# zju3dv/Diffuman4D

Measured on NVIDIA H100. Metric: unet_window_denoise_steps_per_sec, higher is better.
Workload: dtype bf16

## Files before the change

diffuman4d_b200/_lib.py:

```python
from __future__ import annotations

import ctypes as C
import os

_HERE = os.path.dirname(os.path.abspath(__file__))
LIB_PATH = os.path.join(_HERE, "libd4d.so")

EXPORTS = [
    "d4d_last_error", "d4d_version", "d4d_create", "d4d_destroy", "d4d_load_weight", "d4d_finalize_weights",
    "d4d_num_weights", "d4d_weight_key", "d4d_unet_forward", "d4d_profile_forward", "d4d_workspace_bytes", "d4d_forward_launches",
    "d4d_denoise_window", "d4d_denoise_window_dpm", "d4d_assemble_input", "d4d_cfg_ddim_step", "d4d_cfg_dpm_step",
    "d4d_op_gemm", "d4d_op_gemm_kv_scatter", "d4d_op_conv3x3",
    "d4d_op_attention", "d4d_op_groupnorm", "d4d_op_conv3x3_groupnorm", "d4d_op_conv_resample", "d4d_op_layernorm", "d4d_op_pose_conv0", "d4d_op_pose_conv", "d4d_debug_tap", "d4d_exchange_alloc",
    "d4d_exchange_open", "d4d_unet_forward_sharded", "d4d_denoise_window_sharded", "d4d_denoise_window_dpm_sharded",
    "d4d_window_exchange", "d4d_op_window_scatter", "d4d_denoise_window_unipc", "d4d_cfg_unipc_step",
]


class D4DConfig(C.Structure):
    _fields_ = [
        ("in_channels", C.c_int32), ("out_channels", C.c_int32), ("block_out_channels", C.c_int32 * 4),
        ("layers_per_block", C.c_int32), ("num_heads", C.c_int32 * 4), ("has_attn2", C.c_int32 * 4),
        ("use_linear_projection", C.c_int32), ("norm_num_groups", C.c_int32), ("norm_eps", C.c_float),
        ("flip_sin_to_cos", C.c_int32), ("freq_shift", C.c_float), ("num_3d_attn_blocks", C.c_int32),
        ("enable_tem_embeds", C.c_int32), ("enable_pose_encoder", C.c_int32), ("center_input_sample", C.c_int32),
    ]


class D4DSched(C.Structure):
    _fields_ = [
        ("timesteps_table", C.c_void_p), ("alphas_cumprod", C.c_void_p), ("n_steps", C.c_int32),
        ("num_train_timesteps", C.c_int32), ("final_alpha_cumprod", C.c_float), ("prediction_type", C.c_int32),
        ("clip_sample", C.c_int32), ("clip_sample_range", C.c_float), ("emulate_bf16", C.c_int32),
    ]


class D4DDpmSched(C.Structure):
    _fields_ = [
        ("timesteps_table", C.c_void_p), ("coefs", C.c_void_p), ("n_steps", C.c_int32), ("prediction_type", C.c_int32),
        ("solver_order", C.c_int32), ("final_first_order", C.c_int32), ("emulate_bf16", C.c_int32),
    ]


class D4DUniPCSched(C.Structure):
    _fields_ = [
        ("timesteps_table", C.c_void_p), ("coefs", C.c_void_p), ("n_steps", C.c_int32), ("prediction_type", C.c_int32),
        ("solver_order", C.c_int32), ("emulate_bf16", C.c_int32),
    ]


class D4DError(RuntimeError):
    pass


_lib = None


def lib() -> C.CDLL:
    global _lib
    if _lib is None:
        _lib = _load(LIB_PATH)
    return _lib


def _load(path: str) -> C.CDLL:
    if not os.path.exists(path):
        raise ImportError(
            f"{path} not found: the CUDA extension is the product and there is no CPU fallback. "
            "Build it with `python -m diffuman4d_b200.build`.")
    l = C.CDLL(path)
    vp, i32, i64p, f32, f32p = C.c_void_p, C.c_int, C.POINTER(C.c_int64), C.c_float, C.c_void_p
    l.d4d_last_error.restype = C.c_char_p
    l.d4d_last_error.argtypes = []
    l.d4d_version.restype = C.c_int
    l.d4d_create.argtypes = [C.POINTER(D4DConfig), i32, C.POINTER(vp)]
    l.d4d_destroy.argtypes = [vp]
    l.d4d_destroy.restype = None
    l.d4d_load_weight.argtypes = [vp, C.c_char_p, vp, i64p, i32, i32]
    l.d4d_finalize_weights.argtypes = [vp]
    l.d4d_num_weights.argtypes = [vp]
    l.d4d_weight_key.argtypes = [vp, i32]
    l.d4d_weight_key.restype = C.c_char_p
    l.d4d_unet_forward.argtypes = [vp, vp, vp, vp, C.POINTER(C.c_int32), i32, i32, i32, i32, i32, vp, vp]
    l.d4d_profile_forward.argtypes = [vp, vp, vp, vp, C.POINTER(C.c_int32), i32, i32, i32, i32, i32, vp, vp,
                                      C.POINTER(C.c_float), C.POINTER(C.c_int32), C.POINTER(C.c_double)]
    l.d4d_workspace_bytes.argtypes = [vp, i32, i32, i32, i32, i32, C.POINTER(C.c_size_t)]
    l.d4d_forward_launches.argtypes = [vp, i32, i32, i32, i32, i32, C.POINTER(C.c_int)]
    l.d4d_denoise_window.argtypes = [vp, vp, vp, vp, vp, vp, vp, C.POINTER(D4DSched), f32, i32, i32, i32, i32, i32, vp]
    l.d4d_denoise_window_dpm.argtypes = [vp, vp, vp, vp, vp, vp, vp, C.POINTER(D4DDpmSched), f32, i32, i32, i32, i32, i32,
                                         vp, vp, vp]
    l.d4d_denoise_window_unipc.argtypes = [vp, vp, vp, vp, vp, vp, vp, C.POINTER(D4DUniPCSched), f32, i32, i32, i32, i32,
                                           i32, vp, vp, vp, vp, vp]
    l.d4d_assemble_input.argtypes = [vp, vp, vp, vp, vp, vp, vp, i32, i32, i32, i32, i32, vp, vp, vp]
    l.d4d_cfg_ddim_step.argtypes = [vp, vp, vp, vp, vp, C.POINTER(D4DSched), f32, i32, i32, i32, i32, vp, vp]
    l.d4d_cfg_dpm_step.argtypes = [vp, vp, vp, vp, vp, vp, vp, vp, C.POINTER(D4DDpmSched), f32, i32, i32, i32, i32, vp, vp]
    l.d4d_cfg_unipc_step.argtypes = [vp, vp, vp, vp, vp, vp, vp, vp, vp, vp, C.POINTER(D4DUniPCSched), f32, i32, i32, i32,
                                     i32, vp, vp]
    l.d4d_op_gemm.argtypes = [vp, i32, i32, vp, i32, i32, vp, i32, i32, f32p, vp, i32, i32, vp, i32, vp, i32, i32,
                              i32, f32, i32, vp, i32, vp]
    l.d4d_op_gemm_kv_scatter.argtypes = [vp, i32, i32, vp, i32, i32, vp, i32, i32, i32, C.c_int64, C.c_int64, C.c_int64,
                                         i32, vp, i32, vp]
    l.d4d_op_conv3x3.argtypes = [vp, i32, i32, i32, i32, vp, i32, f32p, vp, i32, vp, i32, vp, i32, vp, vp]
    l.d4d_op_attention.argtypes = [vp, vp, vp, i32, vp, i32, i32, i32, i32, i32, f32, i32, i32, vp]
    l.d4d_op_groupnorm.argtypes = [vp, i32, vp, i32, i32, i32, i32, f32, f32p, f32p, i32, vp, vp, vp]
    l.d4d_op_conv3x3_groupnorm.argtypes = [vp, i32, i32, i32, i32, vp, i32, f32p, vp, i32, f32, f32p, f32p, i32, vp, vp, vp,
                                           vp]
    l.d4d_op_conv_resample.argtypes = [vp, i32, i32, i32, i32, vp, i32, f32p, i32, i32, i32, vp, vp, vp]
    l.d4d_op_layernorm.argtypes = [vp, i32, i32, f32, f32p, f32p, vp, vp]
    l.d4d_op_pose_conv0.argtypes = [vp, i32, i32, i32, vp, f32p, vp, vp]
    l.d4d_op_pose_conv.argtypes = [vp, i32, i32, i32, i32, vp, f32p, i32, i32, i32, vp, vp]
    l.d4d_debug_tap.argtypes = [vp, vp, vp, vp, C.POINTER(C.c_int32), i32, i32, i32, i32, i32, i32, vp, C.c_char_p,
                                C.POINTER(C.c_int32), vp]
    l.d4d_exchange_alloc.argtypes = [vp, C.c_size_t, vp]
    l.d4d_exchange_open.argtypes = [vp, i32, i32, vp]
    l.d4d_unet_forward_sharded.argtypes = [vp, vp, vp, vp, C.POINTER(C.c_int32), i32, i32, i32, i32, i32, i32, vp, vp]
    l.d4d_denoise_window_sharded.argtypes = [vp, vp, vp, vp, vp, vp, vp, C.POINTER(D4DSched), f32, i32, i32, i32, i32,
                                             i32, i32, vp]
    l.d4d_denoise_window_dpm_sharded.argtypes = [vp, vp, vp, vp, vp, vp, vp, C.POINTER(D4DDpmSched), f32, i32, i32, i32,
                                                 i32, i32, i32, vp, vp, vp]
    l.d4d_window_exchange.argtypes = [vp, vp, vp, vp, vp, i32, i32, i32, i32, vp, vp, vp, vp, vp]
    l.d4d_op_window_scatter.argtypes = [vp, vp, vp, vp, i32, i32, i32, i32, i32, i32, vp, C.c_size_t, vp]
    for name in EXPORTS:
        fn = getattr(l, name)
        if fn.restype is C.c_int or name.startswith("d4d_op_") or name in (
                "d4d_create", "d4d_load_weight", "d4d_finalize_weights", "d4d_unet_forward", "d4d_denoise_window",
                "d4d_denoise_window_dpm", "d4d_exchange_alloc", "d4d_exchange_open", "d4d_unet_forward_sharded",
                "d4d_denoise_window_sharded", "d4d_denoise_window_dpm_sharded", "d4d_window_exchange", "d4d_debug_tap",
                "d4d_denoise_window_unipc"):
            fn.restype = C.c_int
    return l


def check(rc: int, what: str = ""):
    if rc == 0:
        return
    msg = lib().d4d_last_error().decode("utf-8", "replace")
    if rc == 1:
        raise ValueError(f"{what}: {msg}" if what else msg)
    raise D4DError(f"{what}: {msg} (status {rc})" if what else f"{msg} (status {rc})")
```

diffuman4d_b200/csrc/d4d_api.cu:

```cuda
#include <new>
#include <stdexcept>

#include "unet.h"

namespace d4d {
static thread_local std::string g_last_error;
void set_error(const std::string& msg) { g_last_error = msg; }
int nhwc_to_nchw_run(const bf16* x, int ld, int n, int C, int hw, bf16* out, cudaStream_t stream);
}

struct d4d_handle {
  d4d::Model* model;
};

using d4d::bf16;

#define D4D_API_BEGIN try {
#define D4D_API_END                                        \
  }                                                        \
  catch (const std::bad_alloc&) {                          \
    d4d::set_error("out of host memory");                  \
    return 2;                                              \
  }                                                        \
  catch (const std::exception& e) {                        \
    d4d::set_error(std::string("internal error: ") + e.what()); \
    return 2;                                              \
  }

namespace {
struct DeviceGuard {
  int prev = -1;
  bool ok = true;
  explicit DeviceGuard(int dev) {
    if (cudaGetDevice(&prev) != cudaSuccess) { ok = false; prev = -1; }
    if (ok && prev != dev && cudaSetDevice(dev) != cudaSuccess) ok = false;
  }
  ~DeviceGuard() {
    if (prev >= 0) cudaSetDevice(prev);
  }
};

int unet_forward(d4d_handle* h, const void* sample, const int64_t* timestep, const void* skeletons,
                 const int32_t* domain_ids, int n_domains, int B, int F, int F_total, int height, int width, void* out,
                 void* stream) {
  D4D_API_BEGIN
  D4D_REQUIRE(h != nullptr, "null handle");
  DeviceGuard g(h->model->device());
  return h->model->forward(static_cast<const bf16*>(sample), reinterpret_cast<const long long*>(timestep),
                           static_cast<const bf16*>(skeletons), domain_ids, n_domains, B, F, height, width,
                           static_cast<bf16*>(out), static_cast<cudaStream_t>(stream), F_total);
  D4D_API_END
}

int denoise_window(d4d_handle* h, void* latents, const void* pixel_latents, const void* plucker, const void* skeletons,
                   const void* cond_mask, int64_t* timestep_indices, const d4d::WindowStep& step, float guidance_scale,
                   int domain, int F, int F_total, int height, int width, int num_steps, void* stream) {
  D4D_API_BEGIN
  D4D_REQUIRE(h != nullptr && (step.ddim != nullptr || step.dpm != nullptr || step.unipc != nullptr), "null argument");
  DeviceGuard g(h->model->device());
  return h->model->denoise_window(static_cast<bf16*>(latents), static_cast<const bf16*>(pixel_latents),
                                  static_cast<const bf16*>(plucker), static_cast<const bf16*>(skeletons),
                                  static_cast<const bf16*>(cond_mask), reinterpret_cast<long long*>(timestep_indices),
                                  step, guidance_scale, domain, F, height, width, num_steps,
                                  static_cast<cudaStream_t>(stream), F_total);
  D4D_API_END
}

d4d::WindowStep ddim_step(const d4d_sched* sched) {
  d4d::WindowStep s;
  s.ddim = sched;
  return s;
}

d4d::WindowStep dpm_step(const d4d_dpm_sched* sched, void* x0_prev, int32_t* lower_order_nums) {
  d4d::WindowStep s;
  s.dpm = sched; s.x0_prev = static_cast<bf16*>(x0_prev); s.lower_order_nums = lower_order_nums;
  return s;
}
}

extern "C" {

const char* d4d_last_error(void) { return d4d::g_last_error.c_str(); }
int d4d_version(void) { return 107; }

int d4d_create(const d4d_config* cfg, int device, d4d_handle** out) {
  D4D_API_BEGIN
  D4D_REQUIRE(cfg != nullptr && out != nullptr, "null argument");
  *out = nullptr;
  D4D_REQUIRE(cfg->layers_per_block >= 1 && cfg->layers_per_block <= 4, "layers_per_block");
  D4D_REQUIRE(cfg->out_channels >= 1 && cfg->out_channels <= 16, "out_channels must be in [1,16]");
  D4D_REQUIRE(cfg->in_channels >= 1 && cfg->in_channels <= 16, "in_channels must be in [1,16]");
  D4D_REQUIRE(cfg->norm_num_groups >= 1 && cfg->norm_num_groups <= 64, "norm_num_groups");
  for (int i = 0; i < 4; ++i) {
    const int c = cfg->block_out_channels[i], hds = cfg->num_heads[i];
    D4D_REQUIRE(c > 0 && c % 64 == 0, "block_out_channels must be positive multiples of 64");
    D4D_REQUIRE(c % cfg->norm_num_groups == 0, "channels must be divisible by norm_num_groups");
    D4D_REQUIRE(hds > 0 && c % hds == 0, "channels must be divisible by the number of heads");
    D4D_REQUIRE(c / hds <= 192 && (c / hds) % 8 == 0, "head_dim must be a multiple of 8 and <= 192");
  }
  int ndev = 0;
  D4D_CUDA_OK(cudaGetDeviceCount(&ndev));
  D4D_REQUIRE(device >= 0 && device < ndev, "device index out of range");
  cudaDeviceProp prop;
  D4D_CUDA_OK(cudaGetDeviceProperties(&prop, device));
  if (prop.major != 9 || prop.minor != 0) {
    d4d::set_error("libd4d requires an sm_90a (Hopper H100) device; found compute capability " +
                   std::to_string(prop.major) + "." + std::to_string(prop.minor));
    return 2;
  }
  d4d_handle* h = new d4d_handle();
  h->model = new d4d::Model(*cfg, device);
  *out = h;
  return 0;
  D4D_API_END
}

void d4d_destroy(d4d_handle* h) {
  if (!h) return;
  try {
    delete h->model;
  } catch (...) {
  }
  delete h;
}

int d4d_load_weight(d4d_handle* h, const char* key, const void* data, const int64_t* shape, int ndim, int dtype) {
  D4D_API_BEGIN
  D4D_REQUIRE(h != nullptr, "null handle");
  return h->model->load_weight(key, data, shape, ndim, dtype);
  D4D_API_END
}

int d4d_finalize_weights(d4d_handle* h) {
  D4D_API_BEGIN
  D4D_REQUIRE(h != nullptr, "null handle");
  DeviceGuard g(h->model->device());
  return h->model->finalize();
  D4D_API_END
}

int d4d_num_weights(d4d_handle* h) { return h ? static_cast<int>(h->model->keys().size()) : 0; }
const char* d4d_weight_key(d4d_handle* h, int i) {
  if (!h || i < 0 || i >= static_cast<int>(h->model->keys().size())) return nullptr;
  return h->model->keys()[i].c_str();
}

int d4d_unet_forward(d4d_handle* h, const void* sample, const int64_t* timestep, const void* skeletons,
                     const int32_t* domain_ids, int n_domains, int B, int F, int height, int width, void* out,
                     void* stream) {
  return unet_forward(h, sample, timestep, skeletons, domain_ids, n_domains, B, F, 0, height, width, out, stream);
}

int d4d_profile_forward(d4d_handle* h, const void* sample, const int64_t* timestep, const void* skeletons,
                        const int32_t* domain_ids, int n_domains, int B, int F, int height, int width, void* out,
                        void* stream, float* ms_by_kind, int32_t* launches_by_kind, double* flops_by_kind) {
  D4D_API_BEGIN
  D4D_REQUIRE(h != nullptr, "null handle");
  DeviceGuard g(h->model->device());
  return h->model->profile(static_cast<const bf16*>(sample), reinterpret_cast<const long long*>(timestep),
                           static_cast<const bf16*>(skeletons), domain_ids, n_domains, B, F, height, width,
                           static_cast<bf16*>(out), static_cast<cudaStream_t>(stream), ms_by_kind, launches_by_kind,
                           flops_by_kind);
  D4D_API_END
}

int d4d_workspace_bytes(d4d_handle* h, int n_domains, int B, int F, int height, int width, size_t* bytes) {
  D4D_API_BEGIN
  D4D_REQUIRE(h != nullptr && bytes != nullptr, "null argument");
  d4d::Plan* p = h->model->find_plan(n_domains, B, F, height, width);
  *bytes = p ? p->arena_bytes : 0;
  return 0;
  D4D_API_END
}

int d4d_forward_launches(d4d_handle* h, int n_domains, int B, int F, int height, int width, int* launches) {
  D4D_API_BEGIN
  D4D_REQUIRE(h != nullptr && launches != nullptr, "null argument");
  d4d::Plan* p = h->model->find_plan(n_domains, B, F, height, width);
  *launches = p ? p->launches : 0;
  return 0;
  D4D_API_END
}

int d4d_denoise_window(d4d_handle* h, void* latents, const void* pixel_latents, const void* plucker,
                       const void* skeletons, const void* cond_mask, int64_t* timestep_indices, const d4d_sched* sched,
                       float guidance_scale, int domain, int F, int height, int width, int num_steps, void* stream) {
  return denoise_window(h, latents, pixel_latents, plucker, skeletons, cond_mask, timestep_indices, ddim_step(sched),
                        guidance_scale, domain, F, 0, height, width, num_steps, stream);
}

int d4d_denoise_window_dpm(d4d_handle* h, void* latents, const void* pixel_latents, const void* plucker,
                           const void* skeletons, const void* cond_mask, int64_t* timestep_indices,
                           const d4d_dpm_sched* sched, float guidance_scale, int domain, int F, int height, int width,
                           int num_steps, void* x0_prev, int32_t* lower_order_nums, void* stream) {
  return denoise_window(h, latents, pixel_latents, plucker, skeletons, cond_mask, timestep_indices,
                        dpm_step(sched, x0_prev, lower_order_nums), guidance_scale, domain, F, 0, height, width, num_steps,
                        stream);
}

int d4d_denoise_window_unipc(d4d_handle* h, void* latents, const void* pixel_latents, const void* plucker,
                             const void* skeletons, const void* cond_mask, int64_t* timestep_indices,
                             const d4d_unipc_sched* sched, float guidance_scale, int domain, int F, int height, int width,
                             int num_steps, void* x0_prev, void* x0_prev2, void* last_sample, int32_t* lower_order_nums,
                             void* stream) {
  d4d::WindowStep s;
  s.unipc = sched; s.x0_prev = static_cast<bf16*>(x0_prev); s.x0_prev2 = static_cast<bf16*>(x0_prev2);
  s.last_sample = static_cast<bf16*>(last_sample); s.lower_order_nums = lower_order_nums;
  return denoise_window(h, latents, pixel_latents, plucker, skeletons, cond_mask, timestep_indices, s, guidance_scale,
                        domain, F, 0, height, width, num_steps, stream);
}

int d4d_assemble_input(void* latents, const void* pixel_latents, const void* plucker, const void* skel_latents,
                       const void* cond_mask, const int64_t* timestep_indices, const int64_t* timesteps_table,
                       int n_steps, int F, int height, int width, int cfg, void* sample_out, int64_t* timestep_out,
                       void* stream) {
  D4D_API_BEGIN
  D4D_REQUIRE(latents && pixel_latents && plucker && cond_mask && timestep_indices && timesteps_table && sample_out &&
                  timestep_out, "null argument");
  d4d::AssembleArgs a;
  a.latents = static_cast<bf16*>(latents);
  a.pixel = static_cast<const bf16*>(pixel_latents);
  a.plucker = static_cast<const bf16*>(plucker);
  a.skel_latents = static_cast<const bf16*>(skel_latents);
  a.mask = static_cast<const bf16*>(cond_mask);
  a.timestep_indices = reinterpret_cast<const long long*>(timestep_indices);
  a.timesteps_table = reinterpret_cast<const long long*>(timesteps_table);
  a.n_steps = n_steps; a.F = F; a.h = height; a.w = width; a.cfg = cfg;
  a.sample = static_cast<bf16*>(sample_out);
  a.timestep_out = reinterpret_cast<long long*>(timestep_out);
  return d4d::assemble_input_run(a, static_cast<cudaStream_t>(stream));
  D4D_API_END
}

int d4d_cfg_ddim_step(const void* noise, const void* latents, const void* cond_mask, const int64_t* timestep_indices,
                      int64_t* timestep_indices_out, const d4d_sched* sched, float guidance_scale, int cfg, int F,
                      int height, int width, void* latents_out, void* stream) {
  D4D_API_BEGIN
  D4D_REQUIRE(noise && latents && cond_mask && timestep_indices && timestep_indices_out && sched && latents_out,
              "null argument");
  D4D_REQUIRE(timestep_indices != timestep_indices_out, "timestep_indices_out must not alias timestep_indices");
  d4d::DdimArgs d;
  const int hw = height * width;
  d.noise = static_cast<const bf16*>(noise); d.latents = static_cast<const bf16*>(latents);
  d.mask = static_cast<const bf16*>(cond_mask);
  d.timestep_indices = reinterpret_cast<const long long*>(timestep_indices);
  d.timesteps_table = reinterpret_cast<const long long*>(sched->timesteps_table);
  d.alphas_cumprod = sched->alphas_cumprod;
  d.n_steps = sched->n_steps; d.T = sched->num_train_timesteps; d.final_alpha_cumprod = sched->final_alpha_cumprod;
  d.F = F; d.chw = 4 * hw; d.hw = hw; d.cfg = cfg; d.guidance = guidance_scale;
  d.prediction_type = sched->prediction_type; d.clip_sample = sched->clip_sample; d.clip_range = sched->clip_sample_range;
  d.emulate_bf16 = sched->emulate_bf16; d.out = static_cast<bf16*>(latents_out);
  return d4d::cfg_ddim_step_run(d, reinterpret_cast<long long*>(timestep_indices_out), static_cast<cudaStream_t>(stream));
  D4D_API_END
}

int d4d_cfg_dpm_step(const void* noise, const void* latents, const void* cond_mask, const int64_t* timestep_indices,
                     int64_t* timestep_indices_out, void* x0_prev, const int32_t* lower_order_nums,
                     int32_t* lower_order_nums_out, const d4d_dpm_sched* sched, float guidance_scale, int cfg, int F,
                     int height, int width, void* latents_out, void* stream) {
  D4D_API_BEGIN
  D4D_REQUIRE(noise && latents && cond_mask && timestep_indices && timestep_indices_out && x0_prev && lower_order_nums &&
                  lower_order_nums_out && sched && sched->timesteps_table && sched->coefs && latents_out,
              "null argument");
  d4d::DpmArgs d;
  const int hw = height * width;
  d.noise = static_cast<const bf16*>(noise); d.latents = static_cast<const bf16*>(latents);
  d.mask = static_cast<const bf16*>(cond_mask);
  d.timestep_indices = reinterpret_cast<const long long*>(timestep_indices);
  d.coefs = sched->coefs; d.n_steps = sched->n_steps;
  d.F = F; d.chw = 4 * hw; d.hw = hw; d.cfg = cfg; d.guidance = guidance_scale;
  d.prediction_type = sched->prediction_type; d.solver_order = sched->solver_order;
  d.final_first_order = sched->final_first_order; d.emulate_bf16 = sched->emulate_bf16;
  d.x0_prev = static_cast<bf16*>(x0_prev); d.lower_order_nums = lower_order_nums;
  d.lower_order_nums_out = lower_order_nums_out; d.out = static_cast<bf16*>(latents_out);
  return d4d::cfg_dpm_step_run(d, reinterpret_cast<long long*>(timestep_indices_out), static_cast<cudaStream_t>(stream));
  D4D_API_END
}

int d4d_cfg_unipc_step(const void* noise, const void* latents, const void* cond_mask, const int64_t* timestep_indices,
                       int64_t* timestep_indices_out, void* x0_prev, void* x0_prev2, void* last_sample,
                       const int32_t* lower_order_nums, int32_t* lower_order_nums_out, const d4d_unipc_sched* sched,
                       float guidance_scale, int cfg, int F, int height, int width, void* latents_out, void* stream) {
  D4D_API_BEGIN
  D4D_REQUIRE(noise && latents && cond_mask && timestep_indices && timestep_indices_out && x0_prev && last_sample &&
                  lower_order_nums && lower_order_nums_out && sched && sched->timesteps_table && sched->coefs && latents_out,
              "null argument");
  d4d::UniPCArgs d;
  const int hw = height * width;
  d.noise = static_cast<const bf16*>(noise); d.latents = static_cast<const bf16*>(latents);
  d.mask = static_cast<const bf16*>(cond_mask);
  d.timestep_indices = reinterpret_cast<const long long*>(timestep_indices);
  d.coefs = sched->coefs; d.n_steps = sched->n_steps;
  d.F = F; d.chw = 4 * hw; d.hw = hw; d.cfg = cfg; d.guidance = guidance_scale;
  d.prediction_type = sched->prediction_type; d.solver_order = sched->solver_order; d.emulate_bf16 = sched->emulate_bf16;
  d.x0_prev = static_cast<bf16*>(x0_prev); d.x0_prev2 = static_cast<bf16*>(x0_prev2);
  d.last_sample = static_cast<bf16*>(last_sample); d.lower_order_nums = lower_order_nums;
  d.lower_order_nums_out = lower_order_nums_out; d.out = static_cast<bf16*>(latents_out);
  return d4d::cfg_unipc_step_run(d, reinterpret_cast<long long*>(timestep_indices_out), static_cast<cudaStream_t>(stream));
  D4D_API_END
}

int d4d_op_gemm(const void* A, int lda, int K1, const void* A2, int lda2, int K2, const void* W, int M, int N,
                const float* bias, const void* rowvec, int ld_rowvec, int rows_per_image, const void* residual,
                int ld_res, void* out, int ldo, int geglu, int act, float out_scale, int block_n, int64_t* stats,
                int stats_rows, void* stream) {
  D4D_API_BEGIN
  d4d::GemmDesc d;
  d.A = static_cast<const bf16*>(A); d.lda = lda; d.K1 = K1;
  d.A2 = static_cast<const bf16*>(A2); d.lda2 = lda2; d.K2 = K2;
  d.Wt = static_cast<const bf16*>(W); d.M = M; d.N = N; d.bias = bias;
  d.rowvec = static_cast<const bf16*>(rowvec); d.ld_rowvec = ld_rowvec; d.rows_per_image = rows_per_image;
  d.residual = static_cast<const bf16*>(residual); d.ld_res = ld_res;
  d.out = static_cast<bf16*>(out); d.ldo = ldo; d.geglu = geglu; d.act = act; d.out_scale = out_scale; d.block_n = block_n;
  d.stats = reinterpret_cast<long long*>(stats); d.stats_rows = stats_rows;
  D4D_REQUIRE(M > 0, "empty GEMM");
  d4d::GemmLaunch L;
  if (int rc = d4d::gemm_prepare(d, &L)) return rc;
  return d4d::gemm_run(L, static_cast<cudaStream_t>(stream));
  D4D_API_END
}

int d4d_op_gemm_kv_scatter(const void* A, int lda, int K, const void* W, int M, int N, void* out, int ldo, int kv_col0,
                           int kv_ld, int64_t rows_local, int64_t rows_global, int64_t row_offset, int world,
                           void* const* kv_dst, int block_n, void* stream) {
  D4D_API_BEGIN
  D4D_REQUIRE(M > 0, "empty GEMM");
  D4D_REQUIRE(world >= 1 && world <= 8, "K/V scatter: world must be in [1, 8]");
  D4D_REQUIRE(kv_dst != nullptr, "K/V scatter: null destination buffer");
  d4d::GemmDesc d;
  d.A = static_cast<const bf16*>(A); d.lda = lda; d.K1 = K; d.Wt = static_cast<const bf16*>(W); d.M = M; d.N = N;
  d.out = static_cast<bf16*>(out); d.ldo = ldo; d.block_n = block_n;
  d.kv_world = world; d.kv_col0 = kv_col0; d.kv_ld = kv_ld;
  d.kv_rows_local = rows_local; d.kv_rows_global = rows_global; d.kv_row_offset = row_offset;
  for (int r = 0; r < world; ++r) d.kv_dst[r] = static_cast<bf16*>(kv_dst[r]);
  d4d::GemmLaunch L;
  if (int rc = d4d::gemm_prepare(d, &L)) return rc;
  return d4d::gemm_run(L, static_cast<cudaStream_t>(stream));
  D4D_API_END
}

int d4d_op_conv3x3(const void* x_nhwc, int n_img, int H, int W, int Cin, const void* Wt, int Cout, const float* bias,
                   const void* rowvec, int ld_rowvec, const void* residual, int act, void* out, int block_n,
                   int64_t* stats, void* stream) {
  D4D_API_BEGIN
  D4D_REQUIRE(n_img > 0 && H > 0 && W > 0, "empty conv");
  d4d::GemmDesc d;
  d.conv = 1; d.A = static_cast<const bf16*>(x_nhwc); d.n_img = n_img; d.H = H; d.W = W; d.Cin = Cin;
  d.Wt = static_cast<const bf16*>(Wt); d.N = Cout; d.bias = bias;
  d.rowvec = static_cast<const bf16*>(rowvec); d.ld_rowvec = ld_rowvec;
  d.residual = static_cast<const bf16*>(residual); d.ld_res = Cout;
  d.out = static_cast<bf16*>(out); d.ldo = Cout; d.act = act; d.block_n = block_n;
  d.stats = reinterpret_cast<long long*>(stats);
  d4d::GemmLaunch L;
  if (int rc = d4d::gemm_prepare(d, &L)) return rc;
  return d4d::gemm_run(L, static_cast<cudaStream_t>(stream));
  D4D_API_END
}

int d4d_op_attention(const void* q, const void* k, const void* v, int ld_qkv, void* out, int ld_out, int batch, int seq,
                     int heads, int head_dim, float scale, int seq_kv, int ld_kv, void* stream) {
  D4D_API_BEGIN
  d4d::AttnDesc d;
  d.q = static_cast<const bf16*>(q); d.k = static_cast<const bf16*>(k); d.v = static_cast<const bf16*>(v);
  d.ld_qkv = ld_qkv; d.out = static_cast<bf16*>(out); d.ld_out = ld_out;
  d.batch = batch; d.seq = seq; d.heads = heads; d.head_dim = head_dim; d.scale = scale;
  d.seq_kv = seq_kv; d.ld_kv = ld_kv;
  d4d::AttnLaunch L;
  if (int rc = d4d::attn_prepare(d, &L)) return rc;
  return d4d::attn_run(L, static_cast<cudaStream_t>(stream));
  D4D_API_END
}

int d4d_op_groupnorm(const void* x1, int C1, const void* x2, int C2, int n_img, int hw, int groups, float eps,
                     const float* gamma, const float* beta, int silu, void* out, int64_t* stats, void* stream) {
  D4D_API_BEGIN
  D4D_REQUIRE(n_img > 0 && hw > 0 && groups > 0, "empty GroupNorm");
  cudaStream_t st = static_cast<cudaStream_t>(stream);
  if (x2 == nullptr) C2 = 0;
  long long* s1 = reinterpret_cast<long long*>(stats);
  long long* s2 = C2 > 0 ? s1 + static_cast<size_t>(n_img) * C1 * 2 : nullptr;
  if (int rc = d4d::groupnorm_stats_run(static_cast<const bf16*>(x1), C1, n_img, hw, s1, st)) return rc;
  if (C2 > 0) {
    if (int rc = d4d::groupnorm_stats_run(static_cast<const bf16*>(x2), C2, n_img, hw, s2, st)) return rc;
  }
  return d4d::groupnorm_apply_run(static_cast<const bf16*>(x1), C1, s1, static_cast<const bf16*>(x2), C2, s2, n_img, hw, groups,
                                  eps, gamma, beta, silu, static_cast<bf16*>(out), st);
  D4D_API_END
}

int d4d_op_conv_resample(const void* x_nhwc, int n_img, int H, int W, int Cin, const void* Wt, int Cout, const float* bias,
                         int kind, int up_a, int up_b, void* out, int64_t* stats, void* stream) {
  D4D_API_BEGIN
  D4D_REQUIRE(n_img > 0 && H > 0 && W > 0 && kind >= 1 && kind <= 3, "conv_resample arguments");
  d4d::GemmDesc d;
  d.conv = 1; d.conv_kind = kind; d.up_a = up_a; d.up_b = up_b;
  d.A = static_cast<const bf16*>(x_nhwc); d.n_img = n_img; d.H = H; d.W = W; d.Cin = Cin;
  d.Wt = static_cast<const bf16*>(Wt); d.N = Cout; d.bias = bias;
  d.out = static_cast<bf16*>(out); d.ldo = Cout;
  d.stats = reinterpret_cast<long long*>(stats);
  d4d::GemmLaunch L;
  if (int rc = d4d::gemm_prepare(d, &L)) return rc;
  return d4d::gemm_run(L, static_cast<cudaStream_t>(stream));
  D4D_API_END
}

int d4d_op_conv3x3_groupnorm(const void* x_nhwc, int n_img, int H, int W, int Cin, const void* Wt, int Cout, const float* bias,
                             const void* residual, int groups, float eps, const float* gamma, const float* beta, int silu,
                             void* conv_out, void* gn_out, int64_t* stats, void* stream) {
  D4D_API_BEGIN
  D4D_REQUIRE(n_img > 0 && H > 0 && W > 0 && groups > 0, "empty conv");
  D4D_REQUIRE(stats != nullptr, "null statistics workspace");
  cudaStream_t st = static_cast<cudaStream_t>(stream);
  d4d::GemmDesc d;
  d.conv = 1; d.A = static_cast<const bf16*>(x_nhwc); d.n_img = n_img; d.H = H; d.W = W; d.Cin = Cin;
  d.Wt = static_cast<const bf16*>(Wt); d.N = Cout; d.bias = bias;
  d.residual = static_cast<const bf16*>(residual); d.ld_res = Cout;
  d.out = static_cast<bf16*>(conv_out); d.ldo = Cout;
  d.stats = reinterpret_cast<long long*>(stats);
  d4d::GemmLaunch L;
  if (int rc = d4d::gemm_prepare(d, &L)) return rc;
  if (int rc = d4d::gemm_run(L, st)) return rc;
  return d4d::groupnorm_apply_run(static_cast<const bf16*>(conv_out), Cout, d.stats, nullptr, 0, nullptr, n_img, H * W, groups, eps,
                                  gamma, beta, silu, static_cast<bf16*>(gn_out), st);
  D4D_API_END
}

int d4d_op_layernorm(const void* x, int rows, int C, float eps, const float* gamma, const float* beta, void* out,
                     void* stream) {
  D4D_API_BEGIN
  return d4d::layernorm_run(static_cast<const bf16*>(x), rows, C, eps, gamma, beta, static_cast<bf16*>(out),
                            static_cast<cudaStream_t>(stream));
  D4D_API_END
}

int d4d_op_pose_conv0(const void* x_nchw, int n, int H, int W, const void* Wt, const float* bias, void* out_nhwc4,
                      void* stream) {
  D4D_API_BEGIN
  D4D_REQUIRE(n > 0 && H > 0 && W > 0, "empty pose conv");
  return d4d::pose_conv0_run(static_cast<const bf16*>(x_nchw), n, H, W, static_cast<const bf16*>(Wt), bias,
                             static_cast<bf16*>(out_nhwc4), static_cast<cudaStream_t>(stream));
  D4D_API_END
}

int d4d_op_pose_conv(const void* x_nhwc, int n, int Cin, int H, int W, const void* Wt, const float* bias, int Cout,
                     int ksize, int stride, void* out, void* stream) {
  D4D_API_BEGIN
  D4D_REQUIRE(n > 0 && H > 0 && W > 0, "empty pose conv");
  return d4d::pose_conv_run(static_cast<const bf16*>(x_nhwc), n, Cin, H, W, static_cast<const bf16*>(Wt), bias, Cout,
                            ksize, stride, static_cast<bf16*>(out), static_cast<cudaStream_t>(stream));
  D4D_API_END
}

int d4d_debug_tap(d4d_handle* h, const void* sample, const int64_t* timestep, const void* skeletons,
                  const int32_t* domain_ids, int n_domains, int B, int F, int height, int width, int tap, void* out,
                  char* name64, int32_t* dims3, void* stream) {
  D4D_API_BEGIN
  D4D_REQUIRE(h != nullptr, "null handle");
  DeviceGuard g(h->model->device());
  return h->model->debug_tap(static_cast<const bf16*>(sample), reinterpret_cast<const long long*>(timestep),
                             static_cast<const bf16*>(skeletons), domain_ids, n_domains, B, F, height, width, tap,
                             static_cast<bf16*>(out), name64, dims3, static_cast<cudaStream_t>(stream));
  D4D_API_END
}

int d4d_unet_forward_sharded(d4d_handle* h, const void* sample, const int64_t* timestep, const void* skeletons,
                             const int32_t* domain_ids, int n_domains, int B_local, int F_local, int F_total, int height,
                             int width, void* out, void* stream) {
  return unet_forward(h, sample, timestep, skeletons, domain_ids, n_domains, B_local, F_local, F_total, height, width,
                      out, stream);
}

int d4d_denoise_window_sharded(d4d_handle* h, void* latents, const void* pixel_latents, const void* plucker,
                               const void* skeletons, const void* cond_mask, int64_t* timestep_indices,
                               const d4d_sched* sched, float guidance_scale, int domain, int F_local, int F_total,
                               int height, int width, int num_steps, void* stream) {
  return denoise_window(h, latents, pixel_latents, plucker, skeletons, cond_mask, timestep_indices, ddim_step(sched),
                        guidance_scale, domain, F_local, F_total, height, width, num_steps, stream);
}

int d4d_denoise_window_dpm_sharded(d4d_handle* h, void* latents, const void* pixel_latents, const void* plucker,
                                   const void* skeletons, const void* cond_mask, int64_t* timestep_indices,
                                   const d4d_dpm_sched* sched, float guidance_scale, int domain, int F_local, int F_total,
                                   int height, int width, int num_steps, void* x0_prev, int32_t* lower_order_nums,
                                   void* stream) {
  return denoise_window(h, latents, pixel_latents, plucker, skeletons, cond_mask, timestep_indices,
                        dpm_step(sched, x0_prev, lower_order_nums), guidance_scale, domain, F_local, F_total, height,
                        width, num_steps, stream);
}

int d4d_window_exchange(d4d_handle* h, const void* latents_local, const int64_t* timestep_indices_local,
                        const void* x0_prev_local, const int32_t* lower_order_nums_local, int F_local, int F_total,
                        int height, int width, void* latents_out, int64_t* timestep_indices_out, void* x0_prev_out,
                        int32_t* lower_order_nums_out, void* stream) {
  D4D_API_BEGIN
  D4D_REQUIRE(h != nullptr, "null handle");
  DeviceGuard g(h->model->device());
  return h->model->window_exchange(static_cast<const bf16*>(latents_local),
                                   reinterpret_cast<const long long*>(timestep_indices_local),
                                   static_cast<const bf16*>(x0_prev_local), lower_order_nums_local, F_local, F_total, height,
                                   width, static_cast<bf16*>(latents_out), reinterpret_cast<long long*>(timestep_indices_out),
                                   static_cast<bf16*>(x0_prev_out), lower_order_nums_out, static_cast<cudaStream_t>(stream));
  D4D_API_END
}

int d4d_op_window_scatter(const void* latents, const int64_t* timestep_indices, const void* x0_prev,
                          const int32_t* lower_order_nums, int F_local, int F_total, int height, int width, int world,
                          int rank, void* const* dst, size_t dst_bytes, void* stream) {
  D4D_API_BEGIN
  D4D_REQUIRE(world >= 1 && world <= 8, "window scatter: world must be in [1, 8]");
  D4D_REQUIRE(dst != nullptr, "window scatter: null destination buffer");
  D4D_REQUIRE(height > 0 && width > 0, "window scatter: latent height/width");
  d4d::WindowScatterArgs a;
  for (int r = 0; r < 8; ++r) a.dst[r] = r < world ? dst[r] : nullptr;
  a.world = world; a.rank = rank; a.F_local = F_local; a.F_total = F_total;
  a.chw = 4ll * height * width;
  a.latents = static_cast<const bf16*>(latents); a.ts = reinterpret_cast<const long long*>(timestep_indices);
  a.x0_prev = static_cast<const bf16*>(x0_prev); a.lower_order_nums = lower_order_nums;
  return d4d::window_scatter_run(a, dst_bytes, static_cast<cudaStream_t>(stream));
  D4D_API_END
}

int d4d_exchange_alloc(d4d_handle* h, size_t kv_bytes, unsigned char* handles_out) {
  D4D_API_BEGIN
  D4D_REQUIRE(h != nullptr, "null handle");
  DeviceGuard g(h->model->device());
  return h->model->exchange_alloc(kv_bytes, handles_out);
  D4D_API_END
}

int d4d_exchange_open(d4d_handle* h, int rank, int world, const unsigned char* all_handles) {
  D4D_API_BEGIN
  D4D_REQUIRE(h != nullptr, "null handle");
  DeviceGuard g(h->model->device());
  return h->model->exchange_open(rank, world, all_handles);
  D4D_API_END
}

}
```

diffuman4d_b200/csrc/gemm_wgmma.cu:

```cuda
#include "kernels.h"
#include "wgmma.cuh"

namespace d4d {

namespace {

constexpr int BLOCK_M = 128;
constexpr int BLOCK_K = 64;
constexpr int A_BYTES = BLOCK_M * BLOCK_K * 2;
constexpr int BAR_BYTES = 1024;
constexpr int NUM_THREADS = 384;
constexpr int MAX_SMEM = 227 * 1024;

constexpr int SLAB_COLS = 32;
constexpr int SLAB_BYTES = 64 * SLAB_COLS * 2;

template <int BN, bool kStaged>
struct GemmCfg {
  static constexpr int STAGE_BYTES = A_BYTES + BN * BLOCK_K * 2;
  static constexpr int STAGING_BYTES = kStaged ? 2 * 64 * BN * 2 : 0;
  static constexpr int STAGES_FIT = (MAX_SMEM - 1024 - BAR_BYTES - STAGING_BYTES) / STAGE_BYTES;
  static constexpr int STAGES = STAGES_FIT > 8 ? 8 : STAGES_FIT;
  static constexpr int SMEM = 1024 + BAR_BYTES + STAGES * STAGE_BYTES + STAGING_BYTES;
};

struct TileCoord {
  int m0;
  int n_img0, y0, x0;
  int pa, pb;
};

template <bool kConv>
__device__ __forceinline__ void tile_coords(const GemmKernelArgs& a, int m_tile, TileCoord& t) {
  if (!kConv) {
    t.m0 = m_tile * BLOCK_M;
    t.n_img0 = t.y0 = t.x0 = 0;
    t.pa = t.pb = 0;
  } else {
    const int ph = a.n_phases > 1 ? m_tile / a.tiles_per_phase : 0;
    m_tile -= ph * a.tiles_per_phase;
    t.pa = ph >> 1;
    t.pb = ph & 1;
    int tx = m_tile % a.tiles_x;
    int r = m_tile / a.tiles_x;
    int ty = r % a.tiles_y;
    int tn = r / a.tiles_y;
    t.m0 = 0;
    t.x0 = tx * a.BW;
    t.y0 = ty * a.BH;
    t.n_img0 = tn * a.BN;
  }
}

template <bool kConv>
__device__ __forceinline__ void row_of(const GemmKernelArgs& a, const TileCoord& tc, int rr, long long& row, int& img,
                                       bool& valid) {
  if (!kConv) {
    row = static_cast<long long>(tc.m0) + rr;
    valid = row < a.M;
    img = a.rows_per_image > 0 ? static_cast<int>(row / a.rows_per_image) : 0;
  } else {
    const int bx = rr % a.BW;
    const int r2 = rr / a.BW;
    const int by = r2 % a.BH;
    const int bn = r2 / a.BH;
    const int x = tc.x0 + bx, y = tc.y0 + by, n = tc.n_img0 + bn;
    valid = (x < a.W) && (y < a.H) && (n < a.n_img);
    row = (static_cast<long long>(n) * a.out_H + (y * a.out_sy + a.out_oy + tc.pa)) * a.out_W + (x * a.out_sx + a.out_ox + tc.pb);
    img = n;
  }
}

enum : int { E_BIAS = 1, E_ROWVEC = 2, E_ACT = 4, E_RES = 8, E_STATS = 16, E_KV = 32, E_ALL = 63 };
__host__ __device__ constexpr bool gemm_staged(bool conv, int epi) { return !conv && !(epi & E_KV); }

template <int BN, bool kGeglu, bool kConv, int kEpi>
__global__ void __launch_bounds__(NUM_THREADS, 1)
gemm_wgmma_kernel(const __grid_constant__ CUtensorMap tmap_a, const __grid_constant__ CUtensorMap tmap_a2,
                  const __grid_constant__ CUtensorMap tmap_b, const __grid_constant__ CUtensorMap tmap_c,
                  const __grid_constant__ CUtensorMap tmap_r, const GemmKernelArgs a) {
  constexpr bool kStaged = gemm_staged(kConv, kEpi);
  using Cfg = GemmCfg<BN, kStaged>;
  constexpr int STAGES = Cfg::STAGES;
  extern __shared__ uint8_t smem_raw[];
  uint8_t* smem = reinterpret_cast<uint8_t*>((reinterpret_cast<uintptr_t>(smem_raw) + 1023) & ~uintptr_t(1023));
  uint64_t* full = reinterpret_cast<uint64_t*>(smem);
  uint64_t* empty = full + STAGES;
  uint64_t* res_full = empty + STAGES;
  uint8_t* ring = smem + BAR_BYTES;

  const int warp = __shfl_sync(0xffffffffu, threadIdx.x >> 5, 0);
  const int lane = threadIdx.x & 31;
  const int total_tiles = a.m_tiles * a.n_tiles;

  if (threadIdx.x == 0) {
    tma_prefetch_desc(&tmap_a);
    tma_prefetch_desc(&tmap_b);
    if (a.kb_split < a.k_blocks) tma_prefetch_desc(&tmap_a2);
    for (int i = 0; i < STAGES; ++i) {
      mbar_init(&full[i], 1);
      mbar_init(&empty[i], 2);
    }
    mbar_init(&res_full[0], 1);
    mbar_init(&res_full[1], 1);
    fence_mbar_init();
  }
  __syncthreads();
  pdl_wait();
  pdl_launch_dependents();

  if (warp < 4) {
    setmaxnreg_dec<40>();
    if (threadIdx.x == 0) {
      const uint32_t tx_bytes = A_BYTES + static_cast<uint32_t>(a.block_n) * BLOCK_K * 2;
      int stage = 0;
      uint32_t phase = 0;
      for (int tile = blockIdx.x; tile < total_tiles; tile += gridDim.x) {
        const int m_tile = tile / a.n_tiles;
        const int n_tile = tile % a.n_tiles;
        TileCoord tc;
        tile_coords<kConv>(a, m_tile, tc);
        const int n0 = n_tile * a.block_n;
        for (int kb = 0; kb < a.k_blocks; ++kb) {
          mbar_wait(&empty[stage], phase ^ 1);
          uint8_t* sa = ring + stage * Cfg::STAGE_BYTES;
          uint8_t* sb = sa + A_BYTES;
          mbar_expect_tx(&full[stage], tx_bytes);
          if (!kConv) {
            if (kb < a.kb_split) tma_load_2d(sa, &tmap_a, &full[stage], kb * BLOCK_K, tc.m0);
            else tma_load_2d(sa, &tmap_a2, &full[stage], (kb - a.kb_split) * BLOCK_K, tc.m0);
            tma_load_2d(sb, &tmap_b, &full[stage], kb * BLOCK_K, n0);
          } else {
            const int tap = kb / a.cin_blocks;
            const int cb = kb - tap * a.cin_blocks;
            tma_load_4d(sa, &tmap_a, &full[stage], cb * BLOCK_K, tc.x0 * a.in_stride + a.tap_dx[tap] + tc.pb,
                        tc.y0 * a.in_stride + a.tap_dy[tap] + tc.pa, tc.n_img0);
            tma_load_2d(sb, &tmap_b, &full[stage], tap * a.Cin + cb * BLOCK_K, n0 + (tc.pa * 2 + tc.pb) * a.N);
          }
          if (++stage == STAGES) { stage = 0; phase ^= 1; }
        }
      }
    }
    return;
  }

  setmaxnreg_inc<232>();
  const int wg = (warp >> 2) - 1;
  const int wq = warp & 3;
  const bool wg_leader = (threadIdx.x & 127) == 0;
  const int r_base = wg * 64 + wq * 16 + (lane >> 2);
  const int c_base = 2 * (lane & 3);
  const uint32_t ring_u32 = smem_u32(ring);
  const bool staged = kStaged && a.staged;
  uint8_t* stg = ring + STAGES * Cfg::STAGE_BYTES + wg * 64 * BN * 2;
  const uint32_t stg_u32 = smem_u32(stg) + (r_base - wg * 64) * 64 + c_base * 2;
  const int stg_xor = (lane >> 3) & 3;
  const bool has_res = (kEpi & E_RES) && !kGeglu && a.residual != nullptr;
  const int out_cols = kGeglu ? a.N / 2 : a.N;
  uint32_t res_phase = 0;

  int stage = 0;
  uint32_t phase = 0;
  float acc[BN / 2];
  for (int tile = blockIdx.x; tile < total_tiles; tile += gridDim.x) {
    const int m_tile = tile / a.n_tiles;
    const int n_tile = tile % a.n_tiles;
    TileCoord tc;
    tile_coords<kConv>(a, m_tile, tc);
    const int n0 = n_tile * a.block_n;
    const int ocol0 = kGeglu ? n0 / 2 : n0;
    const int ocols = min(kGeglu ? a.block_n / 2 : a.block_n, out_cols - ocol0);
    const int n_slabs = (ocols + SLAB_COLS - 1) / SLAB_COLS;
    const int orow0 = tc.m0 + wg * 64;
    const bool stg_live = staged && orow0 < a.M;

    int prev_stage = -1;
    for (int kb = 0; kb < a.k_blocks; ++kb) {
      mbar_wait(&full[stage], phase);
      const uint32_t sa = ring_u32 + stage * Cfg::STAGE_BYTES + wg * 64 * 128;
      const uint32_t sb = ring_u32 + stage * Cfg::STAGE_BYTES + A_BYTES;
      const uint64_t adesc = make_wgmma_desc(sa, 16, 1024);
      const uint64_t bdesc = make_wgmma_desc(sb, 16, 1024);
      wgmma_fence();
#pragma unroll
      for (int k = 0; k < BLOCK_K / 16; ++k) {
        const int scale_d = (kb | k) != 0 ? 1 : 0;
        if constexpr (BN == 64) wgmma_ss_n64(acc, adesc + 2 * k, bdesc + 2 * k, scale_d);
        else if constexpr (BN == 128) wgmma_ss_n128(acc, adesc + 2 * k, bdesc + 2 * k, scale_d);
        else if constexpr (BN == 160) wgmma_ss_n160(acc, adesc + 2 * k, bdesc + 2 * k, scale_d);
        else if constexpr (BN == 192) wgmma_ss_n192(acc, adesc + 2 * k, bdesc + 2 * k, scale_d);
        else wgmma_ss_n256(acc, adesc + 2 * k, bdesc + 2 * k, scale_d);
      }
      wgmma_commit();
      if (kb == 0 && staged && wg_leader) {
        bulk_wait_group_read<0>();
        if (has_res && stg_live) {
          mbar_expect_tx(&res_full[wg], n_slabs * SLAB_BYTES);
          for (int s = 0; s < n_slabs; ++s)
            tma_load_2d(stg + s * SLAB_BYTES, &tmap_r, &res_full[wg], ocol0 + s * SLAB_COLS, orow0);
        }
      }
      wgmma_wait<1>();
      if (prev_stage >= 0 && wg_leader) mbar_arrive(&empty[prev_stage]);
      prev_stage = stage;
      if (++stage == STAGES) { stage = 0; phase ^= 1; }
    }
    wgmma_wait<0>();
    wgmma_fence_regs(acc);
    if (wg_leader) mbar_arrive(&empty[prev_stage]);

    long long rows[2];
    int imgs[2];
    bool valid[2];
    row_of<kConv>(a, tc, r_base, rows[0], imgs[0], valid[0]);
    row_of<kConv>(a, tc, r_base + 8, rows[1], imgs[1], valid[1]);
    if (staged) {
      named_barrier_sync(1 + wg, 128);
      if (has_res && stg_live) {
        mbar_wait(&res_full[wg], res_phase);
        res_phase ^= 1;
      }
    }
    auto stg_addr = [&](int j, int h) {
      return stg_u32 + h * 8 * 64 + (j >> 2) * SLAB_BYTES + (((j & 3) ^ stg_xor) << 4);
    };

    if constexpr (kGeglu) {
      const bool has_bias = (kEpi & E_BIAS) && a.bias != nullptr;
#pragma unroll
      for (int p = 0; p < BN / 16; ++p) {
        if (16 * p >= a.block_n || n0 + 16 * p >= a.N) break;
        float2 ba = make_float2(0.f, 0.f), bg = make_float2(0.f, 0.f);
        if (has_bias) {
          ba = __ldg(reinterpret_cast<const float2*>(a.bias + n0 + 16 * p + c_base));
          bg = __ldg(reinterpret_cast<const float2*>(a.bias + n0 + 16 * p + 8 + c_base));
        }
        const int ocol = n0 / 2 + 8 * p + c_base;
#pragma unroll
        for (int h = 0; h < 2; ++h) {
          if (!valid[h]) continue;
          const float a0 = acc[8 * p + 2 * h] + ba.x, a1 = acc[8 * p + 2 * h + 1] + ba.y;
          const float g0 = acc[8 * p + 4 + 2 * h] + bg.x, g1 = acc[8 * p + 4 + 2 * h + 1] + bg.y;
          const uint32_t o = pack_bf16x2(a0 * gelu_erf_f(g0), a1 * gelu_erf_f(g1));
          if (staged) st_shared_u32(stg_addr(p, h), o);
          else *reinterpret_cast<uint32_t*>(a.out + static_cast<size_t>(rows[h]) * a.ldo + ocol) = o;
        }
      }
    } else {
      const bool has_bias = (kEpi & E_BIAS) && a.bias != nullptr, has_rv = (kEpi & E_ROWVEC) && a.rowvec != nullptr;
      const bool has_stats = (kEpi & E_STATS) && a.stats != nullptr;
      const bool has_act = (kEpi & E_ACT) && a.act == 1, has_scale = (kEpi & E_ACT) && a.out_scale != 1.0f;
      const bool has_kv = (kEpi & E_KV) && a.kv_world > 0;
      const long long row0 = __shfl_sync(0xffffffffu, rows[0], 0);
      const bool stats_on = has_stats && __shfl_sync(0xffffffffu, valid[0] ? 1 : 0, 0);
      const int stats_img = !kConv ? static_cast<int>(row0 / a.stats_rows) : __shfl_sync(0xffffffffu, imgs[0], 0);
#pragma unroll
      for (int j = 0; j < BN / 8; ++j) {
        const int cl = 8 * j + c_base;
        const int col = n0 + cl;
        if (8 * j >= a.block_n || n0 + 8 * j >= a.N) break;
        float2 b2 = make_float2(0.f, 0.f);
        if (has_bias) b2 = __ldg(reinterpret_cast<const float2*>(a.bias + col));
        float sv[2][2];
#pragma unroll
        for (int h = 0; h < 2; ++h) {
          sv[h][0] = sv[h][1] = 0.f;
          if (!valid[h]) continue;
          float f0 = acc[4 * j + 2 * h] + b2.x, f1 = acc[4 * j + 2 * h + 1] + b2.y;
          if (has_rv) {
            const float2 v = unpack_bf16x2(*reinterpret_cast<const uint32_t*>(a.rowvec + static_cast<size_t>(imgs[h]) * a.ld_rowvec + col));
            f0 += v.x; f1 += v.y;
          }
          if (has_act) { f0 = silu_f(f0); f1 = silu_f(f1); }
          if (has_scale) { f0 *= a.out_scale; f1 *= a.out_scale; }
          if (has_res) {
            const float2 v = unpack_bf16x2(staged ? ld_shared_u32(stg_addr(j, h))
                                                  : *reinterpret_cast<const uint32_t*>(a.residual + static_cast<size_t>(rows[h]) * a.ld_res + col));
            f0 += v.x; f1 += v.y;
          }
          const uint32_t o = pack_bf16x2(f0, f1);
          if (has_stats) {
            const float2 rv = unpack_bf16x2(o);
            sv[h][0] = rv.x; sv[h][1] = rv.y;
          }
          if (has_kv && col >= a.kv_col0) {
            const long long half = rows[h] / a.kv_rows_local;
            const long long grow = half * a.kv_rows_global + a.kv_row_offset + (rows[h] - half * a.kv_rows_local);
            const size_t off = static_cast<size_t>(grow) * a.kv_ld + (col - a.kv_col0);
#pragma unroll 1
            for (int rk = 0; rk < a.kv_world; ++rk) *reinterpret_cast<uint32_t*>(a.kv_dst[rk] + off) = o;
          } else if (staged) {
            st_shared_u32(stg_addr(j, h), o);
          } else {
            *reinterpret_cast<uint32_t*>(a.out + static_cast<size_t>(rows[h]) * a.ldo + col) = o;
          }
        }
        if (has_stats) {
          float s0 = sv[0][0] + sv[1][0], s1 = sv[0][1] + sv[1][1];
          float q0 = sv[0][0] * sv[0][0] + sv[1][0] * sv[1][0], q1 = sv[0][1] * sv[0][1] + sv[1][1] * sv[1][1];
#pragma unroll
          for (int m = 4; m < 32; m <<= 1) {
            s0 += __shfl_xor_sync(0xffffffffu, s0, m);
            s1 += __shfl_xor_sync(0xffffffffu, s1, m);
            q0 += __shfl_xor_sync(0xffffffffu, q0, m);
            q1 += __shfl_xor_sync(0xffffffffu, q1, m);
          }
          if (stats_on && lane < 4) {
            unsigned long long* st = reinterpret_cast<unsigned long long*>(a.stats) + (static_cast<size_t>(stats_img) * a.N + col) * 2;
            atomicAdd(st + 0, static_cast<unsigned long long>(__float2ll_rn(s0 * kGnSumScale)));
            atomicAdd(st + 1, static_cast<unsigned long long>(__float2ll_rn(q0 * kGnSqScale)));
            atomicAdd(st + 2, static_cast<unsigned long long>(__float2ll_rn(s1 * kGnSumScale)));
            atomicAdd(st + 3, static_cast<unsigned long long>(__float2ll_rn(q1 * kGnSqScale)));
          }
        }
      }
    }
    if (staged) {
      fence_proxy_async_smem();
      named_barrier_sync(1 + wg, 128);
      if (wg_leader && stg_live) {
        for (int s = 0; s < n_slabs; ++s) tma_store_2d(&tmap_c, stg + s * SLAB_BYTES, ocol0 + s * SLAB_COLS, orow0);
        bulk_commit_group();
      }
    }
  }
  if (staged && wg_leader) bulk_wait_group<0>();
}

}

int gemm_prepare(const GemmDesc& d, GemmLaunch* L) {
  D4D_REQUIRE(d.N % 16 == 0, "GEMM N must be a multiple of 16");
  D4D_REQUIRE(d.out != nullptr && d.A != nullptr && d.Wt != nullptr, "null operand");
  D4D_REQUIRE(d.kv_world >= 0 && d.kv_world <= 8, "K/V scatter: world must be in [1, 8]");
  if (d.kv_world > 0) {
    D4D_REQUIRE(!d.conv && !d.geglu && d.kv_col0 >= 0 && d.kv_col0 < d.N && d.kv_col0 % 16 == 0 && d.kv_ld % 8 == 0 &&
                d.kv_ld >= d.N - d.kv_col0, "K/V scatter arguments");
    for (int r = 0; r < d.kv_world; ++r) D4D_REQUIRE(d.kv_dst[r] != nullptr, "K/V scatter: null destination buffer");
    D4D_REQUIRE(d.kv_rows_local > 0 && d.M % d.kv_rows_local == 0, "K/V scatter: M must be a multiple of rows_local");
    D4D_REQUIRE(d.kv_row_offset >= 0 && d.kv_row_offset + d.kv_rows_local <= d.kv_rows_global,
                "K/V scatter: row_offset + rows_local exceeds rows_global");
  }
  GemmKernelArgs& a = L->args;
  memset(&a, 0, sizeof(a));
  int dev = 0, sms = 0;
  D4D_CUDA_OK(cudaGetDevice(&dev));
  D4D_CUDA_OK(cudaDeviceGetAttribute(&sms, cudaDevAttrMultiProcessorCount, dev));
  int bn = d.block_n;
  if (bn <= 0) {
    const long long rows = d.conv ? static_cast<long long>(d.n_img) * d.H * d.W : d.M;
    const long long m_tiles_est = (rows + BLOCK_M - 1) / BLOCK_M;
    long long best_cost = -1;
    for (int c : {64, 128, 160, 192, 256}) {
      if (d.geglu && c % 64 != 0) continue;
      const long long tiles = m_tiles_est * ((d.N + c - 1) / c);
      const long long waves = (tiles + sms - 1) / sms;
      const long long cost = waves * (c + 64) + (static_cast<long long>((d.N + c - 1) / c) * c - d.N) / 4;
      if (best_cost < 0 || cost <= best_cost) { best_cost = cost; bn = c; }
    }
  }
  D4D_REQUIRE(bn >= 16 && bn <= 256 && bn % 16 == 0 && (d.block_n <= 0 || d.N % bn == 0), "no valid block_n");
  a.block_n = bn;
  a.n_tiles = (d.N + bn - 1) / bn;
  a.N = d.N;
  a.bias = d.bias;
  a.rowvec = d.rowvec;
  a.ld_rowvec = d.ld_rowvec;
  a.rows_per_image = d.rows_per_image;
  a.residual = d.residual;
  a.ld_res = d.ld_res;
  a.out = d.out;
  a.ldo = d.ldo;
  a.geglu = d.geglu;
  a.act = d.act;
  a.out_scale = d.out_scale;
  a.stats = d.stats;
  a.stats_rows = d.stats_rows > 0 ? d.stats_rows : 1;
  D4D_REQUIRE(d.stats == nullptr || (!d.geglu && d.kv_world == 0), "GroupNorm statistics: plain / conv epilogue only");
  D4D_REQUIRE(d.stats == nullptr || d.conv || (d.stats_rows > 0 && d.stats_rows % 32 == 0), "statistics need rows-per-image % 32 == 0");
  D4D_REQUIRE(d.stats == nullptr || d.conv || d.M % d.stats_rows == 0, "statistics need M % rows-per-image == 0");
  a.kv_world = d.kv_world;
  a.kv_col0 = d.kv_col0;
  a.kv_ld = d.kv_ld;
  a.kv_rows_local = d.kv_rows_local > 0 ? d.kv_rows_local : 1;
  a.kv_rows_global = d.kv_rows_global;
  a.kv_row_offset = d.kv_row_offset;
  for (int i = 0; i < 8; ++i) a.kv_dst[i] = d.kv_dst[i];
  D4D_REQUIRE(d.ldo % 8 == 0 && (d.residual == nullptr || d.ld_res % 8 == 0) &&
              (d.rowvec == nullptr || d.ld_rowvec % 8 == 0), "leading dimensions must be multiples of 8");

  if (!d.conv) {
    D4D_REQUIRE(d.K1 > 0 && d.K1 % 8 == 0 && d.K2 % 8 == 0, "K must be a multiple of 8");
    D4D_REQUIRE(d.A2 == nullptr || d.K1 % BLOCK_K == 0, "two-source GEMM needs K1 % 64 == 0");
    a.mode = 0;
    a.M = d.M;
    a.m_tiles = (d.M + BLOCK_M - 1) / BLOCK_M;
    a.kb_split = (d.K1 + BLOCK_K - 1) / BLOCK_K;
    const int kb2 = d.A2 ? (d.K2 + BLOCK_K - 1) / BLOCK_K : 0;
    a.k_blocks = a.kb_split + kb2;
    const int K = d.K1 + (d.A2 ? d.K2 : 0);
    if (int rc = make_tmap_2d(&L->tmap_a, d.A, d.M, d.K1, d.lda, BLOCK_K, BLOCK_M, 128)) return rc;
    if (d.A2) {
      if (int rc = make_tmap_2d(&L->tmap_a2, d.A2, d.M, d.K2, d.lda2, BLOCK_K, BLOCK_M, 128)) return rc;
    } else {
      L->tmap_a2 = L->tmap_a;
    }
    if (int rc = make_tmap_2d(&L->tmap_b, d.Wt, d.N, K, K, BLOCK_K, bn, 128)) return rc;
    const auto aligned16 = [](const void* p) { return (reinterpret_cast<uintptr_t>(p) & 15) == 0; };
    a.staged = d.kv_world == 0 && (d.geglu ? bn % (2 * SLAB_COLS) : bn % SLAB_COLS) == 0 && aligned16(d.out) &&
               (d.residual == nullptr || aligned16(d.residual));
    L->tmap_c = L->tmap_r = L->tmap_a;
    if (a.staged) {
      if (int rc = make_tmap_2d(&L->tmap_c, d.out, d.M, d.geglu ? d.N / 2 : d.N, d.ldo, SLAB_COLS, 64, 64)) return rc;
      if (d.residual && !d.geglu)
        if (int rc = make_tmap_2d(&L->tmap_r, d.residual, d.M, d.N, d.ld_res, SLAB_COLS, 64, 64)) return rc;
    }
  } else {
    D4D_REQUIRE(d.Cin % 8 == 0, "conv Cin must be a multiple of 8");
    D4D_REQUIRE(d.conv_kind >= 0 && d.conv_kind <= 3, "conv_kind");
    D4D_REQUIRE(d.conv_kind != 1 || (d.H % 2 == 0 && d.W % 2 == 0), "stride-2 conv needs even H, W");
    a.mode = 1;
    a.n_img = d.n_img; a.Cin = d.Cin;
    a.in_stride = 1; a.out_sy = a.out_sx = 1; a.out_oy = a.out_ox = 0;
    a.n_phases = 1;
    if (d.conv_kind >= 2) {
      const int pa = d.conv_kind == 3 ? 0 : d.up_a, pb = d.conv_kind == 3 ? 0 : d.up_b;
      a.n_taps = 4;
      for (int t = 0; t < 4; ++t) {
        a.tap_dy[t] = static_cast<signed char>((t >> 1) + pa - 1);
        a.tap_dx[t] = static_cast<signed char>((t & 1) + pb - 1);
      }
      a.H = d.H; a.W = d.W; a.out_H = 2 * d.H; a.out_W = 2 * d.W;
      a.out_sy = a.out_sx = 2; a.out_oy = pa; a.out_ox = pb;
      if (d.conv_kind == 3) a.n_phases = 4;
    } else {
      a.n_taps = 9;
      for (int t = 0; t < 9; ++t) {
        a.tap_dy[t] = static_cast<signed char>(t / 3 - 1);
        a.tap_dx[t] = static_cast<signed char>(t % 3 - 1);
      }
      if (d.conv_kind == 1) { a.in_stride = 2; a.H = d.H / 2; a.W = d.W / 2; }
      else { a.H = d.H; a.W = d.W; }
      a.out_H = a.H; a.out_W = a.W;
    }
    a.M = d.n_img * a.H * a.W;
    a.cin_blocks = (d.Cin + BLOCK_K - 1) / BLOCK_K;
    a.k_blocks = a.n_taps * a.cin_blocks;
    a.kb_split = a.k_blocks;
    int bw = 16; while (bw > a.W) bw >>= 1;
    int bh = 128 / bw; while (bh > a.H && bh > 1) bh >>= 1;
    int bnimg = 128 / (bw * bh);
    D4D_REQUIRE(bw * bh * bnimg == 128 && bnimg <= 256, "conv tile shape");
    D4D_REQUIRE(d.stats == nullptr || (bw * bh) % 32 == 0, "statistics need 32-row warps inside one image");
    a.BW = bw; a.BH = bh; a.BN = bnimg;
    a.tiles_x = (a.W + bw - 1) / bw;
    a.tiles_y = (a.H + bh - 1) / bh;
    const int tiles_n = (d.n_img + bnimg - 1) / bnimg;
    a.tiles_per_phase = a.tiles_x * a.tiles_y * tiles_n;
    a.m_tiles = a.tiles_per_phase * a.n_phases;
    a.M *= a.n_phases;
    if (int rc = make_tmap_nhwc(&L->tmap_a, d.A, d.n_img, d.H, d.W, d.Cin, BLOCK_K, bw, bh, bnimg, 128, a.in_stride)) return rc;
    L->tmap_a2 = L->tmap_c = L->tmap_r = L->tmap_a;
    const uint64_t kw = static_cast<uint64_t>(a.n_taps) * d.Cin;
    if (int rc = make_tmap_2d(&L->tmap_b, d.Wt, static_cast<uint64_t>(d.N) * a.n_phases, kw, kw, BLOCK_K, bn, 128)) return rc;
  }
  const int total = a.m_tiles * a.n_tiles;
  L->grid = total < sms ? total : sms;
  return 0;
}

namespace {

using GemmKernelFn = void (*)(const CUtensorMap, const CUtensorMap, const CUtensorMap, const CUtensorMap,
                              const CUtensorMap, const GemmKernelArgs);
struct GemmVariant {
  int bn;
  bool geglu, conv;
  int epi;
  GemmKernelFn fn;
  int smem;
};
#define D4D_GV(BN, G, C, E) {BN, G, C, E, gemm_wgmma_kernel<BN, G, C, E>, GemmCfg<BN, gemm_staged(C, E)>::SMEM}
#define D4D_GV_PLAIN(BN)                                                                                              \
                                         \
  D4D_GV(BN, false, false, 0), D4D_GV(BN, false, false, E_BIAS), D4D_GV(BN, false, false, E_BIAS | E_RES),           \
  D4D_GV(BN, false, false, E_BIAS | E_RES | E_STATS), D4D_GV(BN, false, false, E_ALL)
#define D4D_GV_CONV(BN)                                                                                               \
                                                            \
  D4D_GV(BN, false, true, E_BIAS | E_ROWVEC | E_STATS), D4D_GV(BN, false, true, E_BIAS | E_RES | E_STATS),           \
  D4D_GV(BN, false, true, E_BIAS | E_STATS), D4D_GV(BN, false, true, E_ALL)
const GemmVariant kGemmVariants[] = {
    D4D_GV_PLAIN(128), D4D_GV_CONV(128), D4D_GV(128, true, false, E_BIAS),
    D4D_GV_PLAIN(160), D4D_GV_CONV(160),
    D4D_GV_PLAIN(192),
    D4D_GV_PLAIN(256), D4D_GV_CONV(256), D4D_GV(256, true, false, E_BIAS),
    D4D_GV(64, false, false, E_ALL), D4D_GV(64, false, true, E_ALL), D4D_GV(64, true, false, E_BIAS),
};
#undef D4D_GV_CONV
#undef D4D_GV_PLAIN
#undef D4D_GV
constexpr int kNumGemmVariants = sizeof(kGemmVariants) / sizeof(kGemmVariants[0]);

int gemm_variant_at(const GemmKernelArgs& a, int bn) {
  const bool conv = a.mode != 0, geglu = a.geglu != 0;
  int need = 0;
  if (a.bias) need |= E_BIAS;
  if (!geglu) {
    if (a.rowvec) need |= E_ROWVEC;
    if (a.act == 1 || a.out_scale != 1.0f) need |= E_ACT;
    if (a.residual) need |= E_RES;
    if (a.stats) need |= E_STATS;
    if (a.kv_world > 0) need |= E_KV;
  }
  int generic = -1;
  for (int i = 0; i < kNumGemmVariants; ++i) {
    const GemmVariant& v = kGemmVariants[i];
    if (v.bn != bn || v.geglu != geglu || v.conv != conv) continue;
    if (v.epi == need) return i;
    if ((v.epi & need) == need && (generic < 0 || v.epi == E_ALL)) generic = i;
  }
  return generic;
}

int gemm_variant_of(const GemmKernelArgs& a) {
  for (int bn : {64, 128, 160, 192, 256}) {
    if (bn < a.block_n) continue;
    const int vi = gemm_variant_at(a, bn);
    if (vi >= 0) return vi;
  }
  return -1;
}

}

int gemm_run(const GemmLaunch& L, cudaStream_t stream) {
  static PerDeviceOnce attr_once[kNumGemmVariants];
  const int vi = gemm_variant_of(L.args);
  D4D_REQUIRE(vi >= 0, "no GEMM kernel instantiation covers this launch");
  const GemmVariant& v = kGemmVariants[vi];
  if (int rc = ensure_dyn_smem(v.fn, v.smem, attr_once[vi])) return rc;
  D4D_CUDA_OK(launch_pdl(v.fn, dim3(L.grid), dim3(NUM_THREADS), v.smem, stream, L.tmap_a, L.tmap_a2, L.tmap_b, L.tmap_c, L.tmap_r,
                         L.args));
  D4D_CUDA_OK(cudaGetLastError());
  return 0;
}

double gemm_flops(const GemmLaunch& L) {
  return 2.0 * static_cast<double>(L.args.M) * L.args.N * (static_cast<double>(L.args.k_blocks) * BLOCK_K);
}

}
```

diffuman4d_b200/csrc/kernels.h:

```cpp
#pragma once
#include <cstdlib>
#include <mutex>
#include <utility>
#include <string.h>

#include "common.cuh"

namespace d4d {

constexpr float kGnSumScale = 268435456.f;
constexpr float kGnSqScale = 16777216.f;

struct GemmKernelArgs {
  int M, N, k_blocks, block_n, n_tiles, m_tiles;
  int mode;
  int kb_split;
  int H, W, n_img, Cin, cin_blocks, BW, BH, BN, tiles_x, tiles_y;
  int n_taps, in_stride, out_sy, out_sx, out_oy, out_ox, out_H, out_W;
  int n_phases, tiles_per_phase;
  signed char tap_dy[9], tap_dx[9];
  const float* bias;
  const bf16* rowvec;
  int ld_rowvec, rows_per_image;
  const bf16* residual;
  int ld_res;
  bf16* out;
  int ldo;
  int staged;
  int geglu;
  int act;
  float out_scale;
  long long* stats;
  int stats_rows;
  int kv_world, kv_col0, kv_ld;
  long long kv_rows_local, kv_rows_global, kv_row_offset;
  bf16* kv_dst[8];
};

struct GemmDesc {
  const bf16* A = nullptr;
  int lda = 0, K1 = 0;
  const bf16* A2 = nullptr;
  int lda2 = 0, K2 = 0;
  const bf16* Wt = nullptr;
  int M = 0, N = 0;
  const float* bias = nullptr;
  const bf16* rowvec = nullptr;
  int ld_rowvec = 0, rows_per_image = 0;
  const bf16* residual = nullptr;
  int ld_res = 0;
  bf16* out = nullptr;
  int ldo = 0;
  int geglu = 0;
  int act = 0;
  float out_scale = 1.0f;
  int block_n = 0;
  long long* stats = nullptr;
  int stats_rows = 0;
  int kv_world = 0, kv_col0 = 0, kv_ld = 0;
  long long kv_rows_local = 0, kv_rows_global = 0, kv_row_offset = 0;
  bf16* kv_dst[8] = {nullptr, nullptr, nullptr, nullptr, nullptr, nullptr, nullptr, nullptr};
  int conv = 0, n_img = 0, H = 0, W = 0, Cin = 0;
  int conv_kind = 0, up_a = 0, up_b = 0;
};

struct GemmLaunch {
  CUtensorMap tmap_a, tmap_a2, tmap_b, tmap_c, tmap_r;
  GemmKernelArgs args;
  int grid;
};

int gemm_prepare(const GemmDesc& d, GemmLaunch* L);
int gemm_run(const GemmLaunch& L, cudaStream_t stream);
double gemm_flops(const GemmLaunch& L);

struct AttnDesc {
  const bf16* q = nullptr;
  const bf16* k = nullptr;
  const bf16* v = nullptr;
  int ld_qkv = 0;
  bf16* out = nullptr;
  int ld_out = 0;
  int batch = 0, seq = 0, heads = 0, head_dim = 0;
  int seq_kv = 0;
  int ld_kv = 0;
  float scale = 0.f;
};
struct AttnLaunch {
  CUtensorMap tmap_q, tmap_k, tmap_v;
  AttnDesc d;
  int grid_x, grid_y;
  int variant;
};
int attn_prepare(const AttnDesc& d, AttnLaunch* L);
int attn_run(const AttnLaunch& L, cudaStream_t stream);
double attn_flops(const AttnDesc& d);

int groupnorm_stats_run(const bf16* x, int C, int n_img, int hw, long long* stats, cudaStream_t stream);
int groupnorm_apply_run(const bf16* x1, int C1, const long long* stats1, const bf16* x2, int C2, const long long* stats2, int n_img,
                        int hw, int groups, float eps, const float* gamma, const float* beta, int silu, bf16* out,
                        cudaStream_t stream);
int layernorm_run(const bf16* x, int rows, int C, float eps, const float* gamma, const float* beta, bf16* out,
                  cudaStream_t stream);

int sinusoid_run(const float* pos, int n, int dim, int flip, float freq_shift, bf16* out, cudaStream_t stream);
int sinusoid_i64_run(const long long* pos, int n, int dim, int flip, float freq_shift, bf16* out, cudaStream_t stream);
int silu_run(const bf16* x, long long n, bf16* out, cudaStream_t stream);
int im2col_nchw_run(const bf16* x, int n, int Cin, int H, int W, int cin_pad, int KP, bf16* out, cudaStream_t stream);
int nhwc_to_nchw_run(const bf16* x, int ld, int n, int C, int hw, bf16* out, cudaStream_t stream);
int pose_conv0_run(const bf16* x_nchw, int n, int H, int W, const bf16* w, const float* bias, bf16* out_nhwc4,
                   cudaStream_t stream);
int pose_conv_run(const bf16* x, int n, int Cin, int H, int W, const bf16* w, const float* bias, int Cout, int ksize,
                  int stride, bf16* out_nhwc, cudaStream_t stream);
int im2col_nhwc_run(const bf16* x, int n, int H, int W, int C, int ksize, int stride, bf16* out, cudaStream_t stream);

struct AssembleArgs {
  bf16* latents;
  const bf16* pixel;
  const bf16* plucker;
  const bf16* skel_latents;
  const bf16* mask;
  const long long* timestep_indices;
  const long long* timesteps_table;
  int n_steps;
  int F, h, w, cfg;
  bf16* sample;
  long long* timestep_out;
};
int assemble_input_run(const AssembleArgs& a, cudaStream_t stream);

struct DdimArgs {
  const bf16* noise;
  const bf16* latents;
  const bf16* mask;
  const long long* timestep_indices;
  const long long* timesteps_table;
  const float* alphas_cumprod;
  int n_steps, T;
  float final_alpha_cumprod;
  int F, chw, hw, cfg;
  float guidance;
  int prediction_type;
  int clip_sample;
  float clip_range;
  int emulate_bf16;
  bf16* out;
};
int cfg_ddim_step_run(const DdimArgs& a, long long* ts_out, cudaStream_t stream);

constexpr int kDpmCoefs = 6;
struct DpmArgs {
  const bf16* noise;
  const bf16* latents;
  const bf16* mask;
  const long long* timestep_indices;
  const float* coefs;
  int n_steps;
  int F, chw, hw, cfg;
  float guidance;
  int prediction_type;
  int solver_order;
  int final_first_order;
  int emulate_bf16;
  bf16* x0_prev;
  const int* lower_order_nums;
  int* lower_order_nums_out;
  bf16* out;
};
int cfg_dpm_step_run(const DpmArgs& a, long long* ts_out, cudaStream_t stream);

constexpr int kUniPCCoefs = 14;
struct UniPCArgs {
  const bf16* noise;
  const bf16* latents;
  const bf16* mask;
  const long long* timestep_indices;
  const float* coefs;
  int n_steps;
  int F, chw, hw, cfg;
  float guidance;
  int prediction_type;
  int solver_order;
  int emulate_bf16;
  bf16* x0_prev;
  bf16* x0_prev2;
  bf16* last_sample;
  const int* lower_order_nums;
  int* lower_order_nums_out;
  bf16* out;
};
int cfg_unipc_step_run(const UniPCArgs& a, long long* ts_out, cudaStream_t stream);

struct KvFlagArgs {
  unsigned int* flags[8];
  int rank, world;
  unsigned int epoch;
  int slot;
};
int kv_signal_run(const KvFlagArgs& a, cudaStream_t stream);
int kv_wait_run(const KvFlagArgs& a, cudaStream_t stream);

struct WindowResultLayout {
  size_t x0, ts, lon, bytes;
};
inline WindowResultLayout window_result_layout(long long F_total, long long chw, bool dpm) {
  WindowResultLayout L;
  const size_t rows = static_cast<size_t>(F_total) * static_cast<size_t>(chw) * 2;
  L.x0 = rows;
  L.ts = dpm ? 2 * rows : rows;
  L.lon = L.ts + static_cast<size_t>(F_total) * 8;
  L.bytes = L.lon + (dpm ? static_cast<size_t>(F_total) * 4 : 0);
  return L;
}
struct WindowScatterArgs {
  void* dst[8];
  int world, rank, F_local, F_total;
  long long chw;
  const bf16* latents;
  const long long* ts;
  const bf16* x0_prev;
  const int* lower_order_nums;
};
int window_scatter_run(const WindowScatterArgs& a, size_t dst_bytes, cudaStream_t stream);

struct PerDeviceOnce {
  std::once_flag flag[64];
};
template <typename F>
inline int ensure_dyn_smem(F func, int bytes, PerDeviceOnce& once) {
  int dev = 0;
  D4D_CUDA_OK(cudaGetDevice(&dev));
  if (dev < 0 || dev >= 64) return 0;
  cudaError_t err = cudaSuccess;
  std::call_once(once.flag[dev], [&] { err = cudaFuncSetAttribute(func, cudaFuncAttributeMaxDynamicSharedMemorySize, bytes); });
  D4D_CUDA_OK(err);
  return 0;
}

inline bool pdl_enabled() { return false; }
template <typename... KArgs, typename... Args>
inline cudaError_t launch_pdl(void (*kernel)(KArgs...), dim3 grid, dim3 block, size_t smem, cudaStream_t stream, Args&&... args) {
  cudaLaunchConfig_t cfg = {};
  cfg.gridDim = grid;
  cfg.blockDim = block;
  cfg.dynamicSmemBytes = smem;
  cfg.stream = stream;
  cudaLaunchAttribute attr[1];
  attr[0].id = cudaLaunchAttributeProgrammaticStreamSerialization;
  attr[0].val.programmaticStreamSerializationAllowed = pdl_enabled() ? 1 : 0;
  cfg.attrs = attr;
  cfg.numAttrs = 1;
  return cudaLaunchKernelEx(&cfg, kernel, std::forward<Args>(args)...);
}

}
```

include/d4d.h:

```cpp
#ifndef D4D_H_
#define D4D_H_

#include <stddef.h>
#include <stdint.h>

#ifdef __cplusplus
extern "C" {
#endif

typedef struct d4d_handle d4d_handle;

typedef struct d4d_config {
  int32_t in_channels;
  int32_t out_channels;
  int32_t block_out_channels[4];
  int32_t layers_per_block;
  int32_t num_heads[4];
  int32_t has_attn2[4];
  int32_t use_linear_projection;
  int32_t norm_num_groups;
  float norm_eps;
  int32_t flip_sin_to_cos;
  float freq_shift;
  int32_t num_3d_attn_blocks;
  int32_t enable_tem_embeds;
  int32_t enable_pose_encoder;
  int32_t center_input_sample;
} d4d_config;

typedef struct d4d_sched {
  const int64_t* timesteps_table;
  const float* alphas_cumprod;
  int32_t n_steps;
  int32_t num_train_timesteps;
  float final_alpha_cumprod;
  int32_t prediction_type;
  int32_t clip_sample;
  float clip_sample_range;
  int32_t emulate_bf16;
} d4d_sched;

typedef struct d4d_dpm_sched {
  const int64_t* timesteps_table;
  const float* coefs;
  int32_t n_steps;
  int32_t prediction_type;
  int32_t solver_order;
  int32_t final_first_order;
  int32_t emulate_bf16;
} d4d_dpm_sched;

typedef struct d4d_unipc_sched {
  const int64_t* timesteps_table;
  const float* coefs;
  int32_t n_steps;
  int32_t prediction_type;
  int32_t solver_order;
  int32_t emulate_bf16;
} d4d_unipc_sched;

const char* d4d_last_error(void);
int d4d_version(void);

int d4d_create(const d4d_config* cfg, int device, d4d_handle** out);
void d4d_destroy(d4d_handle* h);

int d4d_load_weight(d4d_handle* h, const char* key, const void* data, const int64_t* shape, int ndim, int dtype);
int d4d_finalize_weights(d4d_handle* h);
int d4d_num_weights(d4d_handle* h);
const char* d4d_weight_key(d4d_handle* h, int i);

int d4d_unet_forward(d4d_handle* h, const void* sample, const int64_t* timestep, const void* skeletons,
                     const int32_t* domain_ids, int n_domains, int B, int F, int height, int width, void* out,
                     void* stream);
int d4d_profile_forward(d4d_handle* h, const void* sample, const int64_t* timestep, const void* skeletons,
                        const int32_t* domain_ids, int n_domains, int B, int F, int height, int width, void* out,
                        void* stream, float* ms_by_kind , int32_t* launches_by_kind ,
                        double* flops_by_kind );
int d4d_workspace_bytes(d4d_handle* h, int n_domains, int B, int F, int height, int width, size_t* bytes);
int d4d_forward_launches(d4d_handle* h, int n_domains, int B, int F, int height, int width, int* launches);

int d4d_denoise_window(d4d_handle* h, void* latents, const void* pixel_latents, const void* plucker,
                       const void* skeletons, const void* cond_mask, int64_t* timestep_indices,
                       const d4d_sched* sched, float guidance_scale, int domain, int F, int height, int width,
                       int num_steps, void* stream);
int d4d_denoise_window_dpm(d4d_handle* h, void* latents, const void* pixel_latents, const void* plucker,
                           const void* skeletons, const void* cond_mask, int64_t* timestep_indices,
                           const d4d_dpm_sched* sched, float guidance_scale, int domain, int F, int height, int width,
                           int num_steps, void* x0_prev, int32_t* lower_order_nums, void* stream);

int d4d_denoise_window_unipc(d4d_handle* h, void* latents, const void* pixel_latents, const void* plucker,
                             const void* skeletons, const void* cond_mask, int64_t* timestep_indices,
                             const d4d_unipc_sched* sched, float guidance_scale, int domain, int F, int height, int width,
                             int num_steps, void* x0_prev, void* x0_prev2, void* last_sample, int32_t* lower_order_nums,
                             void* stream);

int d4d_assemble_input(void* latents, const void* pixel_latents, const void* plucker, const void* skel_latents,
                       const void* cond_mask, const int64_t* timestep_indices, const int64_t* timesteps_table,
                       int n_steps, int F, int height, int width, int cfg, void* sample_out, int64_t* timestep_out,
                       void* stream);
int d4d_cfg_ddim_step(const void* noise, const void* latents, const void* cond_mask, const int64_t* timestep_indices,
                      int64_t* timestep_indices_out, const d4d_sched* sched, float guidance_scale, int cfg, int F,
                      int height, int width, void* latents_out, void* stream);
int d4d_cfg_dpm_step(const void* noise, const void* latents, const void* cond_mask, const int64_t* timestep_indices,
                     int64_t* timestep_indices_out, void* x0_prev, const int32_t* lower_order_nums,
                     int32_t* lower_order_nums_out, const d4d_dpm_sched* sched, float guidance_scale, int cfg, int F,
                     int height, int width, void* latents_out, void* stream);
int d4d_cfg_unipc_step(const void* noise, const void* latents, const void* cond_mask, const int64_t* timestep_indices,
                       int64_t* timestep_indices_out, void* x0_prev, void* x0_prev2, void* last_sample,
                       const int32_t* lower_order_nums, int32_t* lower_order_nums_out, const d4d_unipc_sched* sched,
                       float guidance_scale, int cfg, int F, int height, int width, void* latents_out, void* stream);

int d4d_op_gemm(const void* A, int lda, int K1, const void* A2, int lda2, int K2, const void* W, int M, int N,
                const float* bias, const void* rowvec, int ld_rowvec, int rows_per_image, const void* residual,
                int ld_res, void* out, int ldo, int geglu, int act, float out_scale, int block_n, int64_t* stats,
                int stats_rows, void* stream);
int d4d_op_gemm_kv_scatter(const void* A, int lda, int K, const void* W, int M, int N, void* out, int ldo, int kv_col0,
                           int kv_ld, int64_t rows_local, int64_t rows_global, int64_t row_offset, int world,
                           void* const* kv_dst, int block_n, void* stream);
int d4d_op_conv3x3(const void* x_nhwc, int n_img, int H, int W, int Cin, const void* Wt, int Cout, const float* bias,
                   const void* rowvec, int ld_rowvec, const void* residual, int act, void* out, int block_n,
                   int64_t* stats, void* stream);
int d4d_op_attention(const void* q, const void* k, const void* v, int ld_qkv, void* out, int ld_out, int batch,
                     int seq, int heads, int head_dim, float scale, int seq_kv, int ld_kv, void* stream);
int d4d_op_groupnorm(const void* x1, int C1, const void* x2, int C2, int n_img, int hw, int groups, float eps,
                     const float* gamma, const float* beta, int silu, void* out, int64_t* stats, void* stream);
int d4d_op_conv_resample(const void* x_nhwc, int n_img, int H, int W, int Cin, const void* Wt, int Cout, const float* bias,
                         int kind, int up_a, int up_b, void* out, int64_t* stats, void* stream);
int d4d_op_conv3x3_groupnorm(const void* x_nhwc, int n_img, int H, int W, int Cin, const void* Wt, int Cout,
                             const float* bias, const void* residual, int groups, float eps, const float* gamma,
                             const float* beta, int silu, void* conv_out, void* gn_out, int64_t* stats, void* stream);
int d4d_op_layernorm(const void* x, int rows, int C, float eps, const float* gamma, const float* beta, void* out,
                     void* stream);
int d4d_op_pose_conv0(const void* x_nchw, int n, int H, int W, const void* Wt, const float* bias, void* out_nhwc4,
                      void* stream);
int d4d_op_pose_conv(const void* x_nhwc, int n, int Cin, int H, int W, const void* Wt, const float* bias, int Cout,
                     int ksize, int stride, void* out, void* stream);
int d4d_debug_tap(d4d_handle* h, const void* sample, const int64_t* timestep, const void* skeletons,
                  const int32_t* domain_ids, int n_domains, int B, int F, int height, int width, int tap, void* out,
                  char* name64, int32_t* dims3, void* stream);

int d4d_exchange_alloc(d4d_handle* h, size_t kv_bytes, unsigned char* handles_out );
int d4d_exchange_open(d4d_handle* h, int rank, int world, const unsigned char* all_handles );
int d4d_unet_forward_sharded(d4d_handle* h, const void* sample, const int64_t* timestep, const void* skeletons,
                             const int32_t* domain_ids, int n_domains, int B_local, int F_local, int F_total, int height,
                             int width, void* out, void* stream);
int d4d_denoise_window_sharded(d4d_handle* h, void* latents, const void* pixel_latents, const void* plucker,
                               const void* skeletons, const void* cond_mask, int64_t* timestep_indices,
                               const d4d_sched* sched, float guidance_scale, int domain, int F_local, int F_total,
                               int height, int width, int num_steps, void* stream);
int d4d_denoise_window_dpm_sharded(d4d_handle* h, void* latents, const void* pixel_latents, const void* plucker,
                                   const void* skeletons, const void* cond_mask, int64_t* timestep_indices,
                                   const d4d_dpm_sched* sched, float guidance_scale, int domain, int F_local, int F_total,
                                   int height, int width, int num_steps, void* x0_prev, int32_t* lower_order_nums,
                                   void* stream);
int d4d_window_exchange(d4d_handle* h, const void* latents_local, const int64_t* timestep_indices_local,
                        const void* x0_prev_local, const int32_t* lower_order_nums_local, int F_local, int F_total,
                        int height, int width, void* latents_out, int64_t* timestep_indices_out, void* x0_prev_out,
                        int32_t* lower_order_nums_out, void* stream);
int d4d_op_window_scatter(const void* latents, const int64_t* timestep_indices, const void* x0_prev,
                          const int32_t* lower_order_nums, int F_local, int F_total, int height, int width, int world,
                          int rank, void* const* dst, size_t dst_bytes, void* stream);

#ifdef __cplusplus
}
#endif
#endif
```

Before: 13.38.

## Add 256-row conv GEMM tiles and a cost-model tile chooser

Templates the wgmma GEMM kernel on an M multiplier so conv-mode tiles can cover 256 rows. Each consumer warpgroup then issues two wgmma ops per k-step that share the same B operand, which improves weight reuse and raises arithmetic intensity per stage. A new tile chooser picks both block_m and block_n from a cost model that weighs waves, operand traffic and padding waste. The trade-offs are doubled accumulator registers, fewer pipeline stages fitting in shared memory, and possible wave-quantization losses on small convs.

```diff
diff --git a/diffuman4d_b200/_lib.py b/diffuman4d_b200/_lib.py
--- a/diffuman4d_b200/_lib.py
+++ b/diffuman4d_b200/_lib.py
@@ -14,6 +14,7 @@
     "d4d_op_attention", "d4d_op_groupnorm", "d4d_op_conv3x3_groupnorm", "d4d_op_conv_resample", "d4d_op_layernorm", "d4d_op_pose_conv0", "d4d_op_pose_conv", "d4d_debug_tap", "d4d_exchange_alloc",
     "d4d_exchange_open", "d4d_unet_forward_sharded", "d4d_denoise_window_sharded", "d4d_denoise_window_dpm_sharded",
     "d4d_window_exchange", "d4d_op_window_scatter", "d4d_denoise_window_unipc", "d4d_cfg_unipc_step",
+    "d4d_op_conv_tiled", "d4d_conv_tile_choice",
 ]
 
 
@@ -101,6 +102,8 @@
     l.d4d_op_gemm_kv_scatter.argtypes = [vp, i32, i32, vp, i32, i32, vp, i32, i32, i32, C.c_int64, C.c_int64, C.c_int64,
                                          i32, vp, i32, vp]
     l.d4d_op_conv3x3.argtypes = [vp, i32, i32, i32, i32, vp, i32, f32p, vp, i32, vp, i32, vp, i32, vp, vp]
+    l.d4d_op_conv_tiled.argtypes = [vp, i32, i32, i32, i32, vp, i32, f32p, vp, i32, vp, i32, vp, i32, i32, i32, vp, vp]
+    l.d4d_conv_tile_choice.argtypes = [i32, i32, i32, i32, i32, i32, i32, C.POINTER(C.c_int), C.POINTER(C.c_int)]
     l.d4d_op_attention.argtypes = [vp, vp, vp, i32, vp, i32, i32, i32, i32, i32, f32, i32, i32, vp]
     l.d4d_op_groupnorm.argtypes = [vp, i32, vp, i32, i32, i32, i32, f32, f32p, f32p, i32, vp, vp, vp]
     l.d4d_op_conv3x3_groupnorm.argtypes = [vp, i32, i32, i32, i32, vp, i32, f32p, vp, i32, f32, f32p, f32p, i32, vp, vp, vp,
@@ -126,7 +129,7 @@
                 "d4d_create", "d4d_load_weight", "d4d_finalize_weights", "d4d_unet_forward", "d4d_denoise_window",
                 "d4d_denoise_window_dpm", "d4d_exchange_alloc", "d4d_exchange_open", "d4d_unet_forward_sharded",
                 "d4d_denoise_window_sharded", "d4d_denoise_window_dpm_sharded", "d4d_window_exchange", "d4d_debug_tap",
-                "d4d_denoise_window_unipc"):
+                "d4d_denoise_window_unipc", "d4d_conv_tile_choice"):
             fn.restype = C.c_int
     return l
 
diff --git a/diffuman4d_b200/csrc/d4d_api.cu b/diffuman4d_b200/csrc/d4d_api.cu
--- a/diffuman4d_b200/csrc/d4d_api.cu
+++ b/diffuman4d_b200/csrc/d4d_api.cu
@@ -82,7 +82,7 @@
 extern "C" {
 
 const char* d4d_last_error(void) { return d4d::g_last_error.c_str(); }
-int d4d_version(void) { return 107; }
+int d4d_version(void) { return 108; }
 
 int d4d_create(const d4d_config* cfg, int device, d4d_handle** out) {
   D4D_API_BEGIN
@@ -358,6 +358,34 @@
   D4D_API_END
 }
 
+int d4d_op_conv_tiled(const void* x_nhwc, int n_img, int H, int W, int Cin, const void* Wt, int Cout, const float* bias,
+                      const void* rowvec, int ld_rowvec, const void* residual, int act, void* out, int kind, int block_m,
+                      int block_n, int64_t* stats, void* stream) {
+  D4D_API_BEGIN
+  D4D_REQUIRE(n_img > 0 && H > 0 && W > 0 && (kind == 0 || kind == 1 || kind == 3), "conv_tiled arguments");
+  d4d::GemmDesc d;
+  d.conv = 1; d.conv_kind = kind; d.A = static_cast<const bf16*>(x_nhwc); d.n_img = n_img; d.H = H; d.W = W; d.Cin = Cin;
+  d.Wt = static_cast<const bf16*>(Wt); d.N = Cout; d.bias = bias;
+  d.rowvec = static_cast<const bf16*>(rowvec); d.ld_rowvec = ld_rowvec;
+  d.residual = static_cast<const bf16*>(residual); d.ld_res = Cout;
+  d.out = static_cast<bf16*>(out); d.ldo = Cout; d.act = act; d.block_m = block_m; d.block_n = block_n;
+  d.stats = reinterpret_cast<long long*>(stats);
+  d4d::GemmLaunch L;
+  if (int rc = d4d::gemm_prepare(d, &L)) return rc;
+  return d4d::gemm_run(L, static_cast<cudaStream_t>(stream));
+  D4D_API_END
+}
+
+int d4d_conv_tile_choice(int n_img, int H, int W, int Cin, int Cout, int kind, int sms, int* block_m, int* block_n) {
+  D4D_API_BEGIN
+  D4D_REQUIRE(n_img > 0 && H > 0 && W > 0 && Cin > 0 && kind >= 0 && kind <= 3 && sms > 0 && block_m && block_n,
+              "conv_tile_choice arguments");
+  d4d::GemmDesc d;
+  d.conv = 1; d.conv_kind = kind; d.n_img = n_img; d.H = H; d.W = W; d.Cin = Cin; d.N = Cout;
+  return d4d::gemm_choose_tile(d, sms, block_m, block_n);
+  D4D_API_END
+}
+
 int d4d_op_attention(const void* q, const void* k, const void* v, int ld_qkv, void* out, int ld_out, int batch, int seq,
                      int heads, int head_dim, float scale, int seq_kv, int ld_kv, void* stream) {
   D4D_API_BEGIN
diff --git a/diffuman4d_b200/csrc/gemm_wgmma.cu b/diffuman4d_b200/csrc/gemm_wgmma.cu
--- a/diffuman4d_b200/csrc/gemm_wgmma.cu
+++ b/diffuman4d_b200/csrc/gemm_wgmma.cu
@@ -15,9 +15,9 @@
 constexpr int SLAB_COLS = 32;
 constexpr int SLAB_BYTES = 64 * SLAB_COLS * 2;
 
-template <int BN, bool kStaged>
+template <int BN, int MI, bool kStaged>
 struct GemmCfg {
-  static constexpr int STAGE_BYTES = A_BYTES + BN * BLOCK_K * 2;
+  static constexpr int STAGE_BYTES = MI * A_BYTES + BN * BLOCK_K * 2;
   static constexpr int STAGING_BYTES = kStaged ? 2 * 64 * BN * 2 : 0;
   static constexpr int STAGES_FIT = (MAX_SMEM - 1024 - BAR_BYTES - STAGING_BYTES) / STAGE_BYTES;
   static constexpr int STAGES = STAGES_FIT > 8 ? 8 : STAGES_FIT;
@@ -74,13 +74,14 @@
 enum : int { E_BIAS = 1, E_ROWVEC = 2, E_ACT = 4, E_RES = 8, E_STATS = 16, E_KV = 32, E_ALL = 63 };
 __host__ __device__ constexpr bool gemm_staged(bool conv, int epi) { return !conv && !(epi & E_KV); }
 
-template <int BN, bool kGeglu, bool kConv, int kEpi>
+template <int BN, int MI, bool kGeglu, bool kConv, int kEpi>
 __global__ void __launch_bounds__(NUM_THREADS, 1)
 gemm_wgmma_kernel(const __grid_constant__ CUtensorMap tmap_a, const __grid_constant__ CUtensorMap tmap_a2,
                   const __grid_constant__ CUtensorMap tmap_b, const __grid_constant__ CUtensorMap tmap_c,
                   const __grid_constant__ CUtensorMap tmap_r, const GemmKernelArgs a) {
   constexpr bool kStaged = gemm_staged(kConv, kEpi);
-  using Cfg = GemmCfg<BN, kStaged>;
+  static_assert(MI == 1 || (kConv && MI == 2), "256-row tiles: conv mode only (a plain tile is 128 rows, as are its staging slabs)");
+  using Cfg = GemmCfg<BN, MI, kStaged>;
   constexpr int STAGES = Cfg::STAGES;
   extern __shared__ uint8_t smem_raw[];
   uint8_t* smem = reinterpret_cast<uint8_t*>((reinterpret_cast<uintptr_t>(smem_raw) + 1023) & ~uintptr_t(1023));
@@ -112,7 +113,7 @@
   if (warp < 4) {
     setmaxnreg_dec<40>();
     if (threadIdx.x == 0) {
-      const uint32_t tx_bytes = A_BYTES + static_cast<uint32_t>(a.block_n) * BLOCK_K * 2;
+      const uint32_t tx_bytes = MI * A_BYTES + static_cast<uint32_t>(a.block_n) * BLOCK_K * 2;
       int stage = 0;
       uint32_t phase = 0;
       for (int tile = blockIdx.x; tile < total_tiles; tile += gridDim.x) {
@@ -124,7 +125,7 @@
         for (int kb = 0; kb < a.k_blocks; ++kb) {
           mbar_wait(&empty[stage], phase ^ 1);
           uint8_t* sa = ring + stage * Cfg::STAGE_BYTES;
-          uint8_t* sb = sa + A_BYTES;
+          uint8_t* sb = sa + MI * A_BYTES;
           mbar_expect_tx(&full[stage], tx_bytes);
           if (!kConv) {
             if (kb < a.kb_split) tma_load_2d(sa, &tmap_a, &full[stage], kb * BLOCK_K, tc.m0);
@@ -148,12 +149,12 @@
   const int wg = (warp >> 2) - 1;
   const int wq = warp & 3;
   const bool wg_leader = (threadIdx.x & 127) == 0;
-  const int r_base = wg * 64 + wq * 16 + (lane >> 2);
+  const int r_base = wg * 64 * MI + wq * 16 + (lane >> 2);
   const int c_base = 2 * (lane & 3);
   const uint32_t ring_u32 = smem_u32(ring);
   const bool staged = kStaged && a.staged;
   uint8_t* stg = ring + STAGES * Cfg::STAGE_BYTES + wg * 64 * BN * 2;
-  const uint32_t stg_u32 = smem_u32(stg) + (r_base - wg * 64) * 64 + c_base * 2;
+  const uint32_t stg_u32 = smem_u32(stg) + (r_base - wg * 64 * MI) * 64 + c_base * 2;
   const int stg_xor = (lane >> 3) & 3;
   const bool has_res = (kEpi & E_RES) && !kGeglu && a.residual != nullptr;
   const int out_cols = kGeglu ? a.N / 2 : a.N;
@@ -161,7 +162,7 @@
 
   int stage = 0;
   uint32_t phase = 0;
-  float acc[BN / 2];
+  float acc[MI][BN / 2];
   for (int tile = blockIdx.x; tile < total_tiles; tile += gridDim.x) {
     const int m_tile = tile / a.n_tiles;
     const int n_tile = tile % a.n_tiles;
@@ -177,19 +178,23 @@
     int prev_stage = -1;
     for (int kb = 0; kb < a.k_blocks; ++kb) {
       mbar_wait(&full[stage], phase);
-      const uint32_t sa = ring_u32 + stage * Cfg::STAGE_BYTES + wg * 64 * 128;
-      const uint32_t sb = ring_u32 + stage * Cfg::STAGE_BYTES + A_BYTES;
+      const uint32_t sa = ring_u32 + stage * Cfg::STAGE_BYTES + wg * MI * 64 * 128;
+      const uint32_t sb = ring_u32 + stage * Cfg::STAGE_BYTES + MI * A_BYTES;
       const uint64_t adesc = make_wgmma_desc(sa, 16, 1024);
       const uint64_t bdesc = make_wgmma_desc(sb, 16, 1024);
       wgmma_fence();
 #pragma unroll
       for (int k = 0; k < BLOCK_K / 16; ++k) {
         const int scale_d = (kb | k) != 0 ? 1 : 0;
-        if constexpr (BN == 64) wgmma_ss_n64(acc, adesc + 2 * k, bdesc + 2 * k, scale_d);
-        else if constexpr (BN == 128) wgmma_ss_n128(acc, adesc + 2 * k, bdesc + 2 * k, scale_d);
-        else if constexpr (BN == 160) wgmma_ss_n160(acc, adesc + 2 * k, bdesc + 2 * k, scale_d);
-        else if constexpr (BN == 192) wgmma_ss_n192(acc, adesc + 2 * k, bdesc + 2 * k, scale_d);
-        else wgmma_ss_n256(acc, adesc + 2 * k, bdesc + 2 * k, scale_d);
+#pragma unroll
+        for (int mi = 0; mi < MI; ++mi) {
+          const uint64_t ad = adesc + 512 * mi + 2 * k, bd = bdesc + 2 * k;
+          if constexpr (BN == 64) wgmma_ss_n64(acc[mi], ad, bd, scale_d);
+          else if constexpr (BN == 128) wgmma_ss_n128(acc[mi], ad, bd, scale_d);
+          else if constexpr (BN == 160) wgmma_ss_n160(acc[mi], ad, bd, scale_d);
+          else if constexpr (BN == 192) wgmma_ss_n192(acc[mi], ad, bd, scale_d);
+          else wgmma_ss_n256(acc[mi], ad, bd, scale_d);
+        }
       }
       wgmma_commit();
       if (kb == 0 && staged && wg_leader) {
@@ -206,14 +211,10 @@
       if (++stage == STAGES) { stage = 0; phase ^= 1; }
     }
     wgmma_wait<0>();
-    wgmma_fence_regs(acc);
+#pragma unroll
+    for (int mi = 0; mi < MI; ++mi) wgmma_fence_regs(acc[mi]);
     if (wg_leader) mbar_arrive(&empty[prev_stage]);
 
-    long long rows[2];
-    int imgs[2];
-    bool valid[2];
-    row_of<kConv>(a, tc, r_base, rows[0], imgs[0], valid[0]);
-    row_of<kConv>(a, tc, r_base + 8, rows[1], imgs[1], valid[1]);
     if (staged) {
       named_barrier_sync(1 + wg, 128);
       if (has_res && stg_live) {
@@ -225,92 +226,101 @@
       return stg_u32 + h * 8 * 64 + (j >> 2) * SLAB_BYTES + (((j & 3) ^ stg_xor) << 4);
     };
 
-    if constexpr (kGeglu) {
-      const bool has_bias = (kEpi & E_BIAS) && a.bias != nullptr;
-#pragma unroll
-      for (int p = 0; p < BN / 16; ++p) {
-        if (16 * p >= a.block_n || n0 + 16 * p >= a.N) break;
-        float2 ba = make_float2(0.f, 0.f), bg = make_float2(0.f, 0.f);
-        if (has_bias) {
-          ba = __ldg(reinterpret_cast<const float2*>(a.bias + n0 + 16 * p + c_base));
-          bg = __ldg(reinterpret_cast<const float2*>(a.bias + n0 + 16 * p + 8 + c_base));
-        }
-        const int ocol = n0 / 2 + 8 * p + c_base;
-#pragma unroll
-        for (int h = 0; h < 2; ++h) {
-          if (!valid[h]) continue;
-          const float a0 = acc[8 * p + 2 * h] + ba.x, a1 = acc[8 * p + 2 * h + 1] + ba.y;
-          const float g0 = acc[8 * p + 4 + 2 * h] + bg.x, g1 = acc[8 * p + 4 + 2 * h + 1] + bg.y;
-          const uint32_t o = pack_bf16x2(a0 * gelu_erf_f(g0), a1 * gelu_erf_f(g1));
-          if (staged) st_shared_u32(stg_addr(p, h), o);
-          else *reinterpret_cast<uint32_t*>(a.out + static_cast<size_t>(rows[h]) * a.ldo + ocol) = o;
-        }
-      }
-    } else {
-      const bool has_bias = (kEpi & E_BIAS) && a.bias != nullptr, has_rv = (kEpi & E_ROWVEC) && a.rowvec != nullptr;
-      const bool has_stats = (kEpi & E_STATS) && a.stats != nullptr;
-      const bool has_act = (kEpi & E_ACT) && a.act == 1, has_scale = (kEpi & E_ACT) && a.out_scale != 1.0f;
-      const bool has_kv = (kEpi & E_KV) && a.kv_world > 0;
-      const long long row0 = __shfl_sync(0xffffffffu, rows[0], 0);
-      const bool stats_on = has_stats && __shfl_sync(0xffffffffu, valid[0] ? 1 : 0, 0);
-      const int stats_img = !kConv ? static_cast<int>(row0 / a.stats_rows) : __shfl_sync(0xffffffffu, imgs[0], 0);
-#pragma unroll
-      for (int j = 0; j < BN / 8; ++j) {
-        const int cl = 8 * j + c_base;
-        const int col = n0 + cl;
-        if (8 * j >= a.block_n || n0 + 8 * j >= a.N) break;
-        float2 b2 = make_float2(0.f, 0.f);
-        if (has_bias) b2 = __ldg(reinterpret_cast<const float2*>(a.bias + col));
-        float sv[2][2];
-#pragma unroll
-        for (int h = 0; h < 2; ++h) {
-          sv[h][0] = sv[h][1] = 0.f;
-          if (!valid[h]) continue;
-          float f0 = acc[4 * j + 2 * h] + b2.x, f1 = acc[4 * j + 2 * h + 1] + b2.y;
-          if (has_rv) {
-            const float2 v = unpack_bf16x2(*reinterpret_cast<const uint32_t*>(a.rowvec + static_cast<size_t>(imgs[h]) * a.ld_rowvec + col));
-            f0 += v.x; f1 += v.y;
+#pragma unroll
+    for (int mi = 0; mi < MI; ++mi) {
+      float (&accm)[BN / 2] = acc[mi];
+      long long rows[2];
+      int imgs[2];
+      bool valid[2];
+      row_of<kConv>(a, tc, r_base + 64 * mi, rows[0], imgs[0], valid[0]);
+      row_of<kConv>(a, tc, r_base + 64 * mi + 8, rows[1], imgs[1], valid[1]);
+      if constexpr (kGeglu) {
+        const bool has_bias = (kEpi & E_BIAS) && a.bias != nullptr;
+#pragma unroll
+        for (int p = 0; p < BN / 16; ++p) {
+          if (16 * p >= a.block_n || n0 + 16 * p >= a.N) break;
+          float2 ba = make_float2(0.f, 0.f), bg = make_float2(0.f, 0.f);
+          if (has_bias) {
+            ba = __ldg(reinterpret_cast<const float2*>(a.bias + n0 + 16 * p + c_base));
+            bg = __ldg(reinterpret_cast<const float2*>(a.bias + n0 + 16 * p + 8 + c_base));
           }
-          if (has_act) { f0 = silu_f(f0); f1 = silu_f(f1); }
-          if (has_scale) { f0 *= a.out_scale; f1 *= a.out_scale; }
-          if (has_res) {
-            const float2 v = unpack_bf16x2(staged ? ld_shared_u32(stg_addr(j, h))
-                                                  : *reinterpret_cast<const uint32_t*>(a.residual + static_cast<size_t>(rows[h]) * a.ld_res + col));
-            f0 += v.x; f1 += v.y;
-          }
-          const uint32_t o = pack_bf16x2(f0, f1);
-          if (has_stats) {
-            const float2 rv = unpack_bf16x2(o);
-            sv[h][0] = rv.x; sv[h][1] = rv.y;
-          }
-          if (has_kv && col >= a.kv_col0) {
-            const long long half = rows[h] / a.kv_rows_local;
-            const long long grow = half * a.kv_rows_global + a.kv_row_offset + (rows[h] - half * a.kv_rows_local);
-            const size_t off = static_cast<size_t>(grow) * a.kv_ld + (col - a.kv_col0);
-#pragma unroll 1
-            for (int rk = 0; rk < a.kv_world; ++rk) *reinterpret_cast<uint32_t*>(a.kv_dst[rk] + off) = o;
-          } else if (staged) {
-            st_shared_u32(stg_addr(j, h), o);
-          } else {
-            *reinterpret_cast<uint32_t*>(a.out + static_cast<size_t>(rows[h]) * a.ldo + col) = o;
+          const int ocol = n0 / 2 + 8 * p + c_base;
+#pragma unroll
+          for (int h = 0; h < 2; ++h) {
+            if (!valid[h]) continue;
+            const float a0 = accm[8 * p + 2 * h] + ba.x, a1 = accm[8 * p + 2 * h + 1] + ba.y;
+            const float g0 = accm[8 * p + 4 + 2 * h] + bg.x, g1 = accm[8 * p + 4 + 2 * h + 1] + bg.y;
+            const uint32_t o = pack_bf16x2(a0 * gelu_erf_f(g0), a1 * gelu_erf_f(g1));
+            if (staged) st_shared_u32(stg_addr(p, h), o);
+            else *reinterpret_cast<uint32_t*>(a.out + static_cast<size_t>(rows[h]) * a.ldo + ocol) = o;
           }
         }
-        if (has_stats) {
-          float s0 = sv[0][0] + sv[1][0], s1 = sv[0][1] + sv[1][1];
-          float q0 = sv[0][0] * sv[0][0] + sv[1][0] * sv[1][0], q1 = sv[0][1] * sv[0][1] + sv[1][1] * sv[1][1];
-#pragma unroll
-          for (int m = 4; m < 32; m <<= 1) {
-            s0 += __shfl_xor_sync(0xffffffffu, s0, m);
-            s1 += __shfl_xor_sync(0xffffffffu, s1, m);
-            q0 += __shfl_xor_sync(0xffffffffu, q0, m);
-            q1 += __shfl_xor_sync(0xffffffffu, q1, m);
+      } else {
+        const bool has_bias = (kEpi & E_BIAS) && a.bias != nullptr, has_rv = (kEpi & E_ROWVEC) && a.rowvec != nullptr;
+        const bool has_stats = (kEpi & E_STATS) && a.stats != nullptr;
+        const bool has_act = (kEpi & E_ACT) && a.act == 1, has_scale = (kEpi & E_ACT) && a.out_scale != 1.0f;
+        const bool has_kv = (kEpi & E_KV) && a.kv_world > 0;
+        const long long row0 = __shfl_sync(0xffffffffu, rows[0], 0);
+        const bool stats_on = has_stats && __shfl_sync(0xffffffffu, valid[0] ? 1 : 0, 0);
+        const int stats_img = !kConv ? static_cast<int>(row0 / a.stats_rows) : __shfl_sync(0xffffffffu, imgs[0], 0);
+#pragma unroll
+        for (int j = 0; j < BN / 8; ++j) {
+          const int cl = 8 * j + c_base;
+          const int col = n0 + cl;
+          if (8 * j >= a.block_n || n0 + 8 * j >= a.N) break;
+          float2 b2 = make_float2(0.f, 0.f);
+          if (has_bias) b2 = __ldg(reinterpret_cast<const float2*>(a.bias + col));
+          float sv[2][2];
+#pragma unroll
+          for (int h = 0; h < 2; ++h) {
+            sv[h][0] = sv[h][1] = 0.f;
+            if (!valid[h]) continue;
+            float f0 = accm[4 * j + 2 * h] + b2.x, f1 = accm[4 * j + 2 * h + 1] + b2.y;
+            if (has_rv) {
+              const float2 v = unpack_bf16x2(*reinterpret_cast<const uint32_t*>(a.rowvec + static_cast<size_t>(imgs[h]) * a.ld_rowvec + col));
+              f0 += v.x; f1 += v.y;
+            }
+            if (has_act) { f0 = silu_f(f0); f1 = silu_f(f1); }
+            if (has_scale) { f0 *= a.out_scale; f1 *= a.out_scale; }
+            if (has_res) {
+              const float2 v = unpack_bf16x2(staged ? ld_shared_u32(stg_addr(j, h))
+                                                    : *reinterpret_cast<const uint32_t*>(a.residual + static_cast<size_t>(rows[h]) * a.ld_res + col));
+              f0 += v.x; f1 += v.y;
+            }
+            const uint32_t o = pack_bf16x2(f0, f1);
+            if (has_stats) {
+              const float2 rv = unpack_bf16x2(o);
+              sv[h][0] = rv.x; sv[h][1] = rv.y;
+            }
+            if (has_kv && col >= a.kv_col0) {
+              const long long half = rows[h] / a.kv_rows_local;
+              const long long grow = half * a.kv_rows_global + a.kv_row_offset + (rows[h] - half * a.kv_rows_local);
+              const size_t off = static_cast<size_t>(grow) * a.kv_ld + (col - a.kv_col0);
+#pragma unroll 1
+              for (int rk = 0; rk < a.kv_world; ++rk) *reinterpret_cast<uint32_t*>(a.kv_dst[rk] + off) = o;
+            } else if (staged) {
+              st_shared_u32(stg_addr(j, h), o);
+            } else {
+              *reinterpret_cast<uint32_t*>(a.out + static_cast<size_t>(rows[h]) * a.ldo + col) = o;
+            }
           }
-          if (stats_on && lane < 4) {
-            unsigned long long* st = reinterpret_cast<unsigned long long*>(a.stats) + (static_cast<size_t>(stats_img) * a.N + col) * 2;
-            atomicAdd(st + 0, static_cast<unsigned long long>(__float2ll_rn(s0 * kGnSumScale)));
-            atomicAdd(st + 1, static_cast<unsigned long long>(__float2ll_rn(q0 * kGnSqScale)));
-            atomicAdd(st + 2, static_cast<unsigned long long>(__float2ll_rn(s1 * kGnSumScale)));
-            atomicAdd(st + 3, static_cast<unsigned long long>(__float2ll_rn(q1 * kGnSqScale)));
+          if (has_stats) {
+            float s0 = sv[0][0] + sv[1][0], s1 = sv[0][1] + sv[1][1];
+            float q0 = sv[0][0] * sv[0][0] + sv[1][0] * sv[1][0], q1 = sv[0][1] * sv[0][1] + sv[1][1] * sv[1][1];
+#pragma unroll
+            for (int m = 4; m < 32; m <<= 1) {
+              s0 += __shfl_xor_sync(0xffffffffu, s0, m);
+              s1 += __shfl_xor_sync(0xffffffffu, s1, m);
+              q0 += __shfl_xor_sync(0xffffffffu, q0, m);
+              q1 += __shfl_xor_sync(0xffffffffu, q1, m);
+            }
+            if (stats_on && lane < 4) {
+              unsigned long long* st = reinterpret_cast<unsigned long long*>(a.stats) + (static_cast<size_t>(stats_img) * a.N + col) * 2;
+              atomicAdd(st + 0, static_cast<unsigned long long>(__float2ll_rn(s0 * kGnSumScale)));
+              atomicAdd(st + 1, static_cast<unsigned long long>(__float2ll_rn(q0 * kGnSqScale)));
+              atomicAdd(st + 2, static_cast<unsigned long long>(__float2ll_rn(s1 * kGnSumScale)));
+              atomicAdd(st + 3, static_cast<unsigned long long>(__float2ll_rn(q1 * kGnSqScale)));
+            }
           }
         }
       }
@@ -327,6 +337,59 @@
   if (staged && wg_leader) bulk_wait_group<0>();
 }
 
+}
+
+namespace {
+
+void conv_out_grid(const GemmDesc& d, int* oh, int* ow, int* phases) {
+  *oh = d.conv_kind == 1 ? d.H / 2 : d.H;
+  *ow = d.conv_kind == 1 ? d.W / 2 : d.W;
+  *phases = d.conv_kind == 3 ? 4 : 1;
+}
+
+struct ConvTile { int bw, bh, bn_img; long long tiles; };
+ConvTile conv_tile(int rows, int n_img, int oh, int ow) {
+  ConvTile t;
+  t.bw = 16; while (t.bw > ow) t.bw >>= 1;
+  t.bh = rows / t.bw; while (t.bh > oh && t.bh > 1) t.bh >>= 1;
+  t.bn_img = rows / (t.bw * t.bh);
+  t.tiles = static_cast<long long>((ow + t.bw - 1) / t.bw) * ((oh + t.bh - 1) / t.bh) * ((n_img + t.bn_img - 1) / t.bn_img);
+  return t;
+}
+
+}
+
+constexpr int kOperandWeight = 128;
+constexpr int kMinKBlocks256 = 16;
+
+int gemm_choose_tile(const GemmDesc& d, int sms, int* block_m, int* block_n) {
+  D4D_REQUIRE(d.block_m == 0 || d.block_m == 128 || d.block_m == 256, "block_m must be 0 (automatic), 128 or 256");
+  D4D_REQUIRE(d.block_m != 256 || d.conv, "256-row tiles: convolutions only (a plain GEMM stages a 128-row tile for its TMA store)");
+  D4D_REQUIRE(d.block_m != 256 || d.block_n <= 0 || d.block_n == 128 || d.block_n == 160,
+              "256-row tiles run at block_n 128 or 160 (the accumulators of wider tiles do not fit the register file)");
+  int oh = 0, ow = 0, phases = 1;
+  if (d.conv) conv_out_grid(d, &oh, &ow, &phases);
+  D4D_REQUIRE(!d.conv || (d.n_img > 0 && oh > 0 && ow > 0), "empty conv");
+  long long best_cost = -1;
+  for (int r : {128, 256}) {
+    if (d.block_m > 0 ? r != d.block_m : (r == 256 && !d.conv)) continue;
+    const int k_blocks = d.conv ? (d.conv_kind >= 2 ? 4 : 9) * ((d.Cin + BLOCK_K - 1) / BLOCK_K) : 0;
+    const long long m_tiles = d.conv ? conv_tile(r, d.n_img, oh, ow).tiles * phases : (static_cast<long long>(d.M) + r - 1) / r;
+    for (int c : {64, 128, 160, 192, 256}) {
+      if (d.block_n > 0) c = d.block_n;
+      else if (d.geglu && c % 64 != 0) continue;
+      const long long n_tiles = (d.N + c - 1) / c, tiles = m_tiles * n_tiles;
+      const bool fits = r == 128 || ((c == 128 || c == 160) && (d.block_m == 256 || (tiles >= sms && k_blocks >= kMinKBlocks256)));
+      if (fits) {
+        const long long waves = (tiles + sms - 1) / sms;
+        const long long cost = waves * (static_cast<long long>(r) * c + kOperandWeight * (r + c)) + (n_tiles * c - d.N) * (r / 2);
+        if (best_cost < 0 || cost <= best_cost) { best_cost = cost; *block_m = r; *block_n = c; }
+      }
+      if (d.block_n > 0) break;
+    }
+  }
+  D4D_REQUIRE(best_cost >= 0, "no tile for this block_m / block_n");
+  return 0;
 }
 
 int gemm_prepare(const GemmDesc& d, GemmLaunch* L) {
@@ -346,20 +409,12 @@
   int dev = 0, sms = 0;
   D4D_CUDA_OK(cudaGetDevice(&dev));
   D4D_CUDA_OK(cudaDeviceGetAttribute(&sms, cudaDevAttrMultiProcessorCount, dev));
-  int bn = d.block_n;
-  if (bn <= 0) {
-    const long long rows = d.conv ? static_cast<long long>(d.n_img) * d.H * d.W : d.M;
-    const long long m_tiles_est = (rows + BLOCK_M - 1) / BLOCK_M;
-    long long best_cost = -1;
-    for (int c : {64, 128, 160, 192, 256}) {
-      if (d.geglu && c % 64 != 0) continue;
-      const long long tiles = m_tiles_est * ((d.N + c - 1) / c);
-      const long long waves = (tiles + sms - 1) / sms;
-      const long long cost = waves * (c + 64) + (static_cast<long long>((d.N + c - 1) / c) * c - d.N) / 4;
-      if (best_cost < 0 || cost <= best_cost) { best_cost = cost; bn = c; }
-    }
-  }
-  D4D_REQUIRE(bn >= 16 && bn <= 256 && bn % 16 == 0 && (d.block_n <= 0 || d.N % bn == 0), "no valid block_n");
+  D4D_REQUIRE(d.block_n <= 0 || (d.block_n >= 16 && d.block_n <= 256 && d.block_n % 16 == 0 && d.N % d.block_n == 0),
+              "no valid block_n");
+  D4D_REQUIRE(!d.conv || (d.conv_kind >= 0 && d.conv_kind <= 3), "conv_kind");
+  int bm = 0, bn = 0;
+  if (int rc = gemm_choose_tile(d, sms, &bm, &bn)) return rc;
+  a.block_m = bm;
   a.block_n = bn;
   a.n_tiles = (d.N + bn - 1) / bn;
   a.N = d.N;
@@ -417,7 +472,6 @@
     }
   } else {
     D4D_REQUIRE(d.Cin % 8 == 0, "conv Cin must be a multiple of 8");
-    D4D_REQUIRE(d.conv_kind >= 0 && d.conv_kind <= 3, "conv_kind");
     D4D_REQUIRE(d.conv_kind != 1 || (d.H % 2 == 0 && d.W % 2 == 0), "stride-2 conv needs even H, W");
     a.mode = 1;
     a.n_img = d.n_img; a.Cin = d.Cin;
@@ -447,16 +501,14 @@
     a.cin_blocks = (d.Cin + BLOCK_K - 1) / BLOCK_K;
     a.k_blocks = a.n_taps * a.cin_blocks;
     a.kb_split = a.k_blocks;
-    int bw = 16; while (bw > a.W) bw >>= 1;
-    int bh = 128 / bw; while (bh > a.H && bh > 1) bh >>= 1;
-    int bnimg = 128 / (bw * bh);
-    D4D_REQUIRE(bw * bh * bnimg == 128 && bnimg <= 256, "conv tile shape");
+    const ConvTile ct = conv_tile(bm, d.n_img, a.H, a.W);
+    const int bw = ct.bw, bh = ct.bh, bnimg = ct.bn_img;
+    D4D_REQUIRE(bw * bh * bnimg == bm && bnimg <= 256, "conv tile shape");
     D4D_REQUIRE(d.stats == nullptr || (bw * bh) % 32 == 0, "statistics need 32-row warps inside one image");
     a.BW = bw; a.BH = bh; a.BN = bnimg;
     a.tiles_x = (a.W + bw - 1) / bw;
     a.tiles_y = (a.H + bh - 1) / bh;
-    const int tiles_n = (d.n_img + bnimg - 1) / bnimg;
-    a.tiles_per_phase = a.tiles_x * a.tiles_y * tiles_n;
+    a.tiles_per_phase = static_cast<int>(ct.tiles);
     a.m_tiles = a.tiles_per_phase * a.n_phases;
     a.M *= a.n_phases;
     if (int rc = make_tmap_nhwc(&L->tmap_a, d.A, d.n_img, d.H, d.W, d.Cin, BLOCK_K, bw, bh, bnimg, 128, a.in_stride)) return rc;
@@ -474,31 +526,34 @@
 using GemmKernelFn = void (*)(const CUtensorMap, const CUtensorMap, const CUtensorMap, const CUtensorMap,
                               const CUtensorMap, const GemmKernelArgs);
 struct GemmVariant {
-  int bn;
+  int bn, bm;
   bool geglu, conv;
   int epi;
   GemmKernelFn fn;
   int smem;
 };
-#define D4D_GV(BN, G, C, E) {BN, G, C, E, gemm_wgmma_kernel<BN, G, C, E>, GemmCfg<BN, gemm_staged(C, E)>::SMEM}
+#define D4D_GV_M(BN, MI, G, C, E) \
+  {BN, 128 * MI, G, C, E, gemm_wgmma_kernel<BN, MI, G, C, E>, GemmCfg<BN, MI, gemm_staged(C, E)>::SMEM}
+#define D4D_GV(BN, G, C, E) D4D_GV_M(BN, 1, G, C, E)
 #define D4D_GV_PLAIN(BN)                                                                                              \
                                          \
   D4D_GV(BN, false, false, 0), D4D_GV(BN, false, false, E_BIAS), D4D_GV(BN, false, false, E_BIAS | E_RES),           \
   D4D_GV(BN, false, false, E_BIAS | E_RES | E_STATS), D4D_GV(BN, false, false, E_ALL)
-#define D4D_GV_CONV(BN)                                                                                               \
+#define D4D_GV_CONV(BN, MI)                                                                                           \
                                                             \
-  D4D_GV(BN, false, true, E_BIAS | E_ROWVEC | E_STATS), D4D_GV(BN, false, true, E_BIAS | E_RES | E_STATS),           \
-  D4D_GV(BN, false, true, E_BIAS | E_STATS), D4D_GV(BN, false, true, E_ALL)
+  D4D_GV_M(BN, MI, false, true, E_BIAS | E_ROWVEC | E_STATS), D4D_GV_M(BN, MI, false, true, E_BIAS | E_RES | E_STATS), \
+  D4D_GV_M(BN, MI, false, true, E_BIAS | E_STATS), D4D_GV_M(BN, MI, false, true, E_ALL)
 const GemmVariant kGemmVariants[] = {
-    D4D_GV_PLAIN(128), D4D_GV_CONV(128), D4D_GV(128, true, false, E_BIAS),
-    D4D_GV_PLAIN(160), D4D_GV_CONV(160),
+    D4D_GV_PLAIN(128), D4D_GV_CONV(128, 1), D4D_GV_CONV(128, 2), D4D_GV(128, true, false, E_BIAS),
+    D4D_GV_PLAIN(160), D4D_GV_CONV(160, 1), D4D_GV_CONV(160, 2),
     D4D_GV_PLAIN(192),
-    D4D_GV_PLAIN(256), D4D_GV_CONV(256), D4D_GV(256, true, false, E_BIAS),
+    D4D_GV_PLAIN(256), D4D_GV_CONV(256, 1), D4D_GV(256, true, false, E_BIAS),
     D4D_GV(64, false, false, E_ALL), D4D_GV(64, false, true, E_ALL), D4D_GV(64, true, false, E_BIAS),
 };
 #undef D4D_GV_CONV
 #undef D4D_GV_PLAIN
 #undef D4D_GV
+#undef D4D_GV_M
 constexpr int kNumGemmVariants = sizeof(kGemmVariants) / sizeof(kGemmVariants[0]);
 
 int gemm_variant_at(const GemmKernelArgs& a, int bn) {
@@ -515,7 +570,7 @@
   int generic = -1;
   for (int i = 0; i < kNumGemmVariants; ++i) {
     const GemmVariant& v = kGemmVariants[i];
-    if (v.bn != bn || v.geglu != geglu || v.conv != conv) continue;
+    if (v.bn != bn || v.bm != a.block_m || v.geglu != geglu || v.conv != conv) continue;
     if (v.epi == need) return i;
     if ((v.epi & need) == need && (generic < 0 || v.epi == E_ALL)) generic = i;
   }
diff --git a/diffuman4d_b200/csrc/kernels.h b/diffuman4d_b200/csrc/kernels.h
--- a/diffuman4d_b200/csrc/kernels.h
+++ b/diffuman4d_b200/csrc/kernels.h
@@ -13,6 +13,7 @@
 
 struct GemmKernelArgs {
   int M, N, k_blocks, block_n, n_tiles, m_tiles;
+  int block_m;
   int mode;
   int kb_split;
   int H, W, n_img, Cin, cin_blocks, BW, BH, BN, tiles_x, tiles_y;
@@ -55,6 +56,7 @@
   int act = 0;
   float out_scale = 1.0f;
   int block_n = 0;
+  int block_m = 0;
   long long* stats = nullptr;
   int stats_rows = 0;
   int kv_world = 0, kv_col0 = 0, kv_ld = 0;
@@ -70,6 +72,7 @@
   int grid;
 };
 
+int gemm_choose_tile(const GemmDesc& d, int sms, int* block_m, int* block_n);
 int gemm_prepare(const GemmDesc& d, GemmLaunch* L);
 int gemm_run(const GemmLaunch& L, cudaStream_t stream);
 double gemm_flops(const GemmLaunch& L);
diff --git a/include/d4d.h b/include/d4d.h
--- a/include/d4d.h
+++ b/include/d4d.h
@@ -121,6 +121,10 @@
 int d4d_op_conv3x3(const void* x_nhwc, int n_img, int H, int W, int Cin, const void* Wt, int Cout, const float* bias,
                    const void* rowvec, int ld_rowvec, const void* residual, int act, void* out, int block_n,
                    int64_t* stats, void* stream);
+int d4d_op_conv_tiled(const void* x_nhwc, int n_img, int H, int W, int Cin, const void* Wt, int Cout, const float* bias,
+                      const void* rowvec, int ld_rowvec, const void* residual, int act, void* out, int kind, int block_m,
+                      int block_n, int64_t* stats, void* stream);
+int d4d_conv_tile_choice(int n_img, int H, int W, int Cin, int Cout, int kind, int sms, int* block_m, int* block_n);
 int d4d_op_attention(const void* q, const void* k, const void* v, int ld_qkv, void* out, int ld_out, int batch,
                      int seq, int heads, int head_dim, float scale, int seq_kv, int ld_kv, void* stream);
 int d4d_op_groupnorm(const void* x1, int C1, const void* x2, int C2, int n_img, int hw, int groups, float eps,
```

Measured after the change: 14.08, median of 6. 5.2% higher.
